# tsnorri/vcf2multialign

Measured on AMD Instinct MI355X. Metric: aligned A2M Gbases/sec, higher is better.
Workload: dtype u8

## Files before the change

vcf2multialign_amd/csrc/kernels.hpp:

```cpp
#pragma once

#include <hip/hip_runtime.h>
#include <stdint.h>

#ifdef V2M_CHECKED_BUILD
__device__ uint32_t v2m_lds_poison_seed;
#endif

namespace v2m {

typedef uint32_t u32;
typedef uint64_t u64;

constexpr int kWave = 64;
typedef u32 vec4u __attribute__((ext_vector_type(4)));
typedef vec4u vec4u_unaligned8 __attribute__((aligned(8)));

#ifdef V2M_CHECKED_BUILD
__device__ __forceinline__ u32 poison_hash(u32 seed, u32 wg, u32 i)
{
	u32 h = seed ^ (wg * 0x9E3779B1u) ^ (i * 0x85EBCA77u);
	h ^= h >> 15; h *= 0x2C1B3C6Du;
	h ^= h >> 12; h *= 0x297A2D39u;
	h ^= h >> 15;
// ... 741 lines not shown
		}
	}
	for (u32 e = 0; e < 15; ++e) {
		u32 const cg = span_hi + e;
#pragma unroll
		for (int a = 0; a < kA; ++a)
			if (col_ok[a]) emit_guarded(a, cg & 15u, cg);
	}
}
#endif


__device__ __forceinline__ uint4 expand_reference_chunk(
	char const *__restrict__ ref, u32 const *__restrict__ ref_pos, u32 const *__restrict__ aln_pos,
	u32 n_nodes, u32 L, u64 p0, char gap, unsigned char past)
{
	unsigned char bytes[16];
	if (p0 >= L) {
		u32 const w = past * 0x01010101u;
		return make_uint4(w, w, w, w);
	}
	u32 lo = 0, hi = n_nodes;
	while (hi - lo > 1) {
		u32 const mid = lo + (hi - lo) / 2;
		if (aln_pos[mid] <= p0) lo = mid; else hi = mid;
	}
	u32 n = lo;
	u32 a0 = aln_pos[n], r0 = ref_pos[n];
	u32 a1 = (n + 1 < n_nodes) ? aln_pos[n + 1] : 0xFFFFFFFFu;
	u32 r1 = (n + 1 < n_nodes) ? ref_pos[n + 1] : r0;
#pragma unroll
	for (int b = 0; b < 16; ++b) {
		u64 const p = p0 + b;
		unsigned char v = past;
		if (p < L) {
			while (p >= a1) {
				++n;
				a0 = a1; r0 = r1;
				a1 = (n + 1 < n_nodes) ? aln_pos[n + 1] : 0xFFFFFFFFu;
				r1 = (n + 1 < n_nodes) ? ref_pos[n + 1] : r0;
			}
			u32 const off = (u32) p - a0;
			v = (off < r1 - r0) ? (unsigned char) ref[r0 + off] : (unsigned char) gap;
		}
		bytes[b] = v;
	}
	uint4 o;
	o.x = bytes[0] | (bytes[1] << 8) | (bytes[2] << 16) | ((u32) bytes[3] << 24);
	o.y = bytes[4] | (bytes[5] << 8) | (bytes[6] << 16) | ((u32) bytes[7] << 24);
	o.z = bytes[8] | (bytes[9] << 8) | (bytes[10] << 16) | ((u32) bytes[11] << 24);
	o.w = bytes[12] | (bytes[13] << 8) | (bytes[14] << 16) | ((u32) bytes[15] << 24);
	return o;
}

__global__ __launch_bounds__(256) void expand_reference_row_kernel(
	char const *__restrict__ ref, u32 const *__restrict__ ref_pos, u32 const *__restrict__ aln_pos,
	u32 n_nodes, u32 L, u64 n_chunks, uint4 *__restrict__ out, char gap, u32 col_base = 0)
{
	u64 const c = (u64) blockIdx.x * blockDim.x + threadIdx.x;
	if (c >= n_chunks) return;
	u64 const p0 = col_base + c * 16;
	out[c] = expand_reference_chunk(ref, ref_pos, aln_pos, n_nodes, L, p0, gap, 0);
}

struct set_tile_tables {
	u32 const *col_begin;
	u32 const *col_end;
	u32 const *record_offset;
	u32 const *edge_end;
};

__global__ __launch_bounds__(256) void expand_reference_set_kernel(
	char const *__restrict__ ref, u32 const *__restrict__ ref_pos, u32 const *__restrict__ aln_pos,
	u32 n_nodes, set_tile_tables st, u32 n_tiles, u64 n_chunks, uint4 *__restrict__ out, char gap)
{
	u64 const c = (u64) blockIdx.x * blockDim.x + threadIdx.x;
	if (c >= n_chunks) return;
	u32 lo = 0, hi = n_tiles;
	while (hi - lo > 1) {
		u32 const mid = lo + (hi - lo) / 2;
		if ((u64) st.record_offset[mid] <= c * 16) lo = mid; else hi = mid;
	}
	u64 const p0 = (u64) st.col_begin[lo] + (c * 16 - st.record_offset[lo]);
	out[c] = expand_reference_chunk(ref, ref_pos, aln_pos, n_nodes, st.col_end[lo], p0, gap, (unsigned char) gap);
}


struct row_segments {
	u32 const *seg_offsets;
	u32 const *seg_edge_begin;
	u32 const *seg_copy;
	u64 const *assembled;
	u32 assembled_words;
};

__device__ __forceinline__ u64 load_row_word(
	u64 const *__restrict__ paths, u64 words_per_copy, row_segments const &rs, u32 row, u32 s_begin, u32 s_end, u32 wi)
{
	if (s_end - s_begin == 1) {
		u32 const copy = rs.seg_copy[s_begin];
		return (copy == 0xFFFFFFFFu) ? 0 : paths[(u64) copy * words_per_copy + wi];
	}
	return rs.assembled[(u64) row * rs.assembled_words + wi];
}

__global__ __launch_bounds__(256) void assemble_row_bits_kernel(
	u64 const *__restrict__ paths, u64 words_per_copy, row_segments rs, u64 *__restrict__ assembled, u32 n_words, u32 row_base, u32 word_base)
{
	__shared__ unsigned long long acc[256];
	u32 const row = blockIdx.y + row_base;
	u32 const s_begin = rs.seg_offsets[row], s_end = rs.seg_offsets[row + 1];
	if (s_end - s_begin <= 1) return;
	V2M_POISON_LDS(acc);
	u32 const lane = threadIdx.x & 63, wave = threadIdx.x >> 6;
	u32 const w0 = word_base + (blockIdx.x * 4 + wave) * 64;
	acc[threadIdx.x] = 0;
	__syncthreads();
	if (w0 < n_words) {
		u64 const e_lo = (u64) w0 * 64;
		u64 const e_hi = (u64) (w0 + 64 < n_words ? w0 + 64 : n_words) * 64;
		u32 lo = s_begin, hi = s_end;
		while (hi - lo > 1) {
			u32 const mid = lo + (hi - lo) / 2;
			if (rs.seg_edge_begin[mid] <= e_lo) lo = mid; else hi = mid;
		}
		for (u32 s = lo + lane; s < s_end; s += 64) {
			u64 b = rs.seg_edge_begin[s];
			if (b >= e_hi) break;
			u64 e = (s + 1 < s_end) ? rs.seg_edge_begin[s + 1] : ~0ULL;
			u32 const copy = rs.seg_copy[s];
			if (copy == 0xFFFFFFFFu) continue;
			b = b > e_lo ? b : e_lo;
			e = e < e_hi ? e : e_hi;
			if (b >= e) continue;
			u64 const *const column = paths + (u64) copy * words_per_copy;
			for (u64 wi = b >> 6; wi <= (e - 1) >> 6; ++wi) {
				u64 const base = wi * 64;
				u32 const from = b > base ? (u32) (b - base) : 0;
				u32 const to = e < base + 64 ? (u32) (e - base) : 64;
				u64 const mask = (to >= 64 ? ~0ULL : ((1ULL << to) - 1)) & ~((1ULL << from) - 1);
				u64 const v = column[wi] & mask;
				if (v) atomicOr(&acc[wave * 64 + (u32) (wi - w0)], (unsigned long long) v);
			}
		}
	}
	__syncthreads();
	if (w0 + lane < n_words) assembled[(u64) row * rs.assembled_words + w0 + lane] = acc[threadIdx.x];
}

constexpr int kResolveWordsPerThread = 8;
constexpr u32 kResolveQueueShards = 1024;
constexpr u32 kMaxBackWords = 2048;

__device__ __forceinline__ u64 resolve_word_exact(
	u64 const *__restrict__ paths, u64 words_per_copy, row_segments const &rs, u32 row, u32 s_begin, u32 s_end,
	edge_span const *__restrict__ spans, u64 const *__restrict__ overlappable,
	u32 wi, u64 w, u64 ovl_w, u32 *__restrict__ needs_serial, u32 max_back_words)
{
	u64 const ov = w & ovl_w;
	if (0 == ov) return w;
	int const b0 = __builtin_ctzll(ov);
	u32 sw = wi;
	int sb = 0;
	u64 fixed = ~ovl_w & ((1ULL << b0) - 1);
	if (fixed) {
		sb = 63 - __builtin_clzll(fixed);
	} else {
		u32 steps = 0;
		for (;;) {
			if (0 == sw) { sb = 0; break; }
			--sw;
			if (++steps > max_back_words) { atomicOr(&needs_serial[row], 1u); return w; }
			fixed = ~overlappable[sw];
			if (fixed) { sb = 63 - __builtin_clzll(fixed); break; }
		}
	}
	u64 out = (sw == wi) ? (w & ((1ULL << sb) - 1)) : 0;
	u32 cur = 0;
	for (u32 ww = sw; ww <= wi; ++ww) {
		u64 x = (ww == wi) ? w : load_row_word(paths, words_per_copy, rs, row, s_begin, s_end, ww);
		if (ww == sw) x &= ~((1ULL << sb) - 1);
		while (x) {
			constexpr int kBatch = 8;
			edge_span sp[kBatch];
			int bit[kBatch];
			bool has[kBatch];
#pragma unroll
			for (int k = 0; k < kBatch; ++k) {
				has[k] = 0 != x;
				bit[k] = has[k] ? __builtin_ctzll(x) : 0;
				x &= x - 1;
				sp[k] = spans[ww * 64u + bit[k]];
			}
#pragma unroll
			for (int k = 0; k < kBatch; ++k) {
				if (has[k] && sp[k].src >= cur) {
					cur = sp[k].tgt;
					if (ww == wi) out |= 1ULL << bit[k];
				}
			}
		}
	}
	return out;
}

__global__ __launch_bounds__(256) void resolve_effective_edges_kernel(
	u64 const *__restrict__ paths, u64 words_per_copy, u32 n_edges,
	row_segments rs, edge_span const *__restrict__ spans, u64 const *__restrict__ overlappable,
	u32 const *__restrict__ ovl_rank, u64 const *__restrict__ blocker_masks,
	u64 *__restrict__ eff, u32 n_words, u32 eff_words_per_row, u32 row_base, u32 word_base,
	u32 *__restrict__ queue, u32 *__restrict__ queue_counts , u32 shard_capacity, u32 *__restrict__ needs_serial, u32 max_back_words)
{
	u32 const row = blockIdx.x + row_base;
	u32 const shard = (blockIdx.y * gridDim.x + blockIdx.x) % kResolveQueueShards;
	u32 const s_begin = rs.seg_offsets[row], s_end = rs.seg_offsets[row + 1];
	u64 const tail_mask = (n_edges & 63) ? (1ULL << (n_edges & 63)) - 1 : ~0ULL;
	u64 const *row_words = nullptr;
	if (s_end - s_begin == 1) {
		u32 const copy = rs.seg_copy[s_begin];
		if (copy != 0xFFFFFFFFu) row_words = paths + (u64) copy * words_per_copy;
	} else {
		row_words = rs.assembled + (u64) row * rs.assembled_words;
	}
	u32 const w_first = word_base + blockIdx.y * kResolveWordsPerThread * blockDim.x + threadIdx.x;
	u64 w_all[kResolveWordsPerThread], ovl_all[kResolveWordsPerThread], mask_a[kResolveWordsPerThread], mask_b[kResolveWordsPerThread];
	u32 rank_all[kResolveWordsPerThread];
#pragma unroll
	for (int piece = 0; piece < kResolveWordsPerThread; ++piece) {
		u32 const wi = w_first + piece * blockDim.x;
		u32 const wc = wi < n_words ? wi : n_words - 1;
		w_all[piece] = row_words ? row_words[wc] : 0;
		ovl_all[piece] = overlappable[wc];
		rank_all[piece] = ovl_rank[wc];
		if (wi == (n_edges - 1) >> 6) w_all[piece] &= tail_mask;
	}
#pragma unroll
	for (int piece = 0; piece < kResolveWordsPerThread; ++piece) {
		u64 const ov = w_all[piece] & ovl_all[piece], ov2 = ov & (ov - 1);
		auto const entry = [&](u64 m) {
			return m ? rank_all[piece] + (u32) __builtin_popcountll(ovl_all[piece] & ((1ULL << __builtin_ctzll(m)) - 1)) : 0u;
		};
		mask_a[piece] = blocker_masks[entry(ov)];
		mask_b[piece] = blocker_masks[entry(ov2)];
	}
	int const lane = threadIdx.x & 63;
#pragma unroll
	for (int piece = 0; piece < kResolveWordsPerThread; ++piece) {
		u32 const wi = w_first + piece * blockDim.x;
		bool const in_range = wi < n_words;
		u64 const w = w_all[piece], ov = w & ovl_all[piece], ov2 = ov & (ov - 1);
		bool const hard = in_range && ov && ((w & mask_a[piece]) || (ov2 && ((w & mask_b[piece]) || (ov2 & (ov2 - 1)))));
		if (in_range && !hard) eff[(u64) row * eff_words_per_row + wi] = w;
		u64 const hard_lanes = __ballot(hard);
		if (hard_lanes) {
			u32 base = 0;
			if (0 == lane) base = atomicAdd(&queue_counts[shard], (u32) __builtin_popcountll(hard_lanes));
			base = __shfl(base, 0, kWave);
			if (hard) {
				u32 const slot = base + __builtin_amdgcn_mbcnt_hi((u32) (hard_lanes >> 32), __builtin_amdgcn_mbcnt_lo((u32) hard_lanes, 0));
				if (slot < shard_capacity) queue[(u64) shard * shard_capacity + slot] = (row - row_base) * n_words + wi;
				else eff[(u64) row * eff_words_per_row + wi] = resolve_word_exact(paths, words_per_copy, rs, row, s_begin, s_end, spans, overlappable, wi, w, ovl_all[piece], needs_serial, max_back_words);
			}
		}
	}
}

__global__ __launch_bounds__(256) void resolve_queued_words_kernel(
	u64 const *__restrict__ paths, u64 words_per_copy, u32 n_edges,
	row_segments rs, edge_span const *__restrict__ spans, u64 const *__restrict__ overlappable,
	u64 *__restrict__ eff, u32 n_words, u32 eff_words_per_row, u32 row_base,
	u32 const *__restrict__ queue, u32 const *__restrict__ queue_counts, u32 shard_capacity, u32 *__restrict__ needs_serial, u32 max_back_words)
{
	u32 const shard = blockIdx.x % kResolveQueueShards, part = blockIdx.x / kResolveQueueShards, parts = gridDim.x / kResolveQueueShards;
	u32 const n = queue_counts[shard] < shard_capacity ? queue_counts[shard] : shard_capacity;
	u64 const tail_mask = (n_edges & 63) ? (1ULL << (n_edges & 63)) - 1 : ~0ULL;
	for (u32 i = part * blockDim.x + threadIdx.x; i < n; i += parts * blockDim.x) {
		u32 const entry = queue[(u64) shard * shard_capacity + i];
		u32 const row = row_base + entry / n_words, wi = entry % n_words;
		u32 const s_begin = rs.seg_offsets[row], s_end = rs.seg_offsets[row + 1];
		u64 w = load_row_word(paths, words_per_copy, rs, row, s_begin, s_end, wi);
		if (wi == (n_edges - 1) >> 6) w &= tail_mask;
		eff[(u64) row * eff_words_per_row + wi] = resolve_word_exact(paths, words_per_copy, rs, row, s_begin, s_end, spans, overlappable, wi, w, overlappable[wi], needs_serial, max_back_words);
	}
}


__global__ __launch_bounds__(256) void resolve_rows_serial_kernel(
	u64 const *__restrict__ paths, u64 words_per_copy, u32 n_edges,
	row_segments rs, edge_span const *__restrict__ spans,
	u64 *__restrict__ eff, u64 eff_words_per_row, u32 n_rows, u32 const *__restrict__ needs_serial,
	u32 word_begin , u32 word_end)
{
	int const lane = threadIdx.x & 63;
	u32 const row = blockIdx.x * (blockDim.x >> 6) + (threadIdx.x >> 6);
	if (row >= n_rows) return;
	if (needs_serial && 0 == needs_serial[row]) return;

	u32 const s_begin = rs.seg_offsets[row], s_end = rs.seg_offsets[row + 1];
	u32 const n_words = (n_edges + 63) / 64;
	u64 *const eff_row = eff + (u64) row * eff_words_per_row;
	u32 cur = 0;

	for (u32 base = word_begin; base < word_end; base += 64) {
		u32 const wi = base + lane;
		u64 w = 0;
		if (wi < word_end) {
			w = load_row_word(paths, words_per_copy, rs, row, s_begin, s_end, wi);
			if (wi == n_words - 1 && (n_edges & 63))
				w &= (1ULL << (n_edges & 63)) - 1;
		}

		u32 lane_max = 0;
		for (u64 m = w; m; m &= m - 1) {
			u32 const e = wi * 64u + __builtin_ctzll(m);
			u32 const tgt = spans[e].tgt;
			lane_max = tgt > lane_max ? tgt : lane_max;
		}
		u32 incl = lane_max;
#pragma unroll
		for (int d = 1; d < 64; d <<= 1) {
			u32 const o = __shfl_up(incl, d, kWave);
			if (lane >= d) incl = o > incl ? o : incl;
		}
		u32 excl = __shfl_up(incl, 1, kWave);
		if (lane == 0) excl = 0;
		u32 const chunk_max = __shfl(incl, 63, kWave);

		u32 run = excl > cur ? excl : cur;
		bool uncertain = false;
		for (u64 m = w; m; m &= m - 1) {
			u32 const e = wi * 64u + __builtin_ctzll(m);
			edge_span const sp = spans[e];
			uncertain |= sp.src < run;
			run = sp.tgt > run ? sp.tgt : run;
		}

		u64 out = w;
		if (__any(uncertain)) {
			out = 0;
			u32 c = cur;
			u64 busy = __ballot(w != 0);
			while (busy) {
				int const j = __builtin_ctzll(busy);
				busy &= busy - 1;
				if (lane == j) {
					for (u64 m = w; m; m &= m - 1) {
						int const b = __builtin_ctzll(m);
						edge_span const sp = spans[wi * 64u + b];
						if (sp.src >= c) {
							out |= 1ULL << b;
							c = sp.tgt;
						}
					}
				}
				c = __shfl(c, j, kWave);
			}
			cur = c;
		} else {
			cur = chunk_max > cur ? chunk_max : cur;
		}
		if (wi < word_end)
			eff_row[wi] = out;
	}
}


struct tile_tables {
	u32 const *edge_begin;
	u32 const *cross_offsets;
	u32 const *cross_edges;
};

template <typename LabelPtr>
__device__ __forceinline__ void fill_patch_bytes(
	unsigned char *tile, u32 tile_base, u32 aln_begin, u32 label_len, LabelPtr label,
	u32 from, u32 to, u32 start, u32 step, char gap)
{
	for (u32 pos = from + start; pos < to; pos += step) {
		u32 const off = pos - aln_begin;
		tile[pos - tile_base] = (off < label_len) ? (unsigned char) label[off] : (unsigned char) gap;
	}
}

constexpr int kCandLds = 512;
constexpr int kLabelLds = 1024;
constexpr int kGroupRowsLds = 16;
constexpr int kEffWordsLds = kCandLds / 64 + 2;
constexpr int kLongQueueLds = 16;

struct cached_patch {
	unsigned short begin_rel;
	unsigned short span;
	unsigned short label_rel;
	unsigned short label_len;
};

struct patch_cache {
	cached_patch patch[kCandLds];
	u64 eff[kGroupRowsLds][kEffWordsLds];
	unsigned char labels[kLabelLds];
	u32 long_queue[kLongQueueLds];
	u32 long_count;
};

struct tile_job {
	u32 tile_base, tile_end;
	u32 cross_begin, n_cross, range_begin, n_range;
	u32 n_lds;
	u32 w0;
};

__device__ __forceinline__ void load_eff_cache(
	patch_cache &pc, tile_job const &job, u64 const *__restrict__ eff, u64 eff_words_per_row, u32 first_row, u32 n_rows, int t)
{
	if (0 == job.n_lds) return;
	u32 const nw = ((job.range_begin + job.n_lds - 1) >> 6) - job.w0 + 1;
	u32 const rows = n_rows < (u32) kGroupRowsLds ? n_rows : (u32) kGroupRowsLds;
	for (u32 i = t; i < rows * nw; i += kSpliceThreads)
		pc.eff[i / nw][i % nw] = eff[(u64) (first_row + i / nw) * eff_words_per_row + job.w0 + i % nw];
}

template <bool kWindow = false, bool kSet = false>
__device__ __forceinline__ void load_patch_cache(
	patch_cache &pc, tile_job &job, tile_tables const &tt, edge_patch const *__restrict__ patches, char const *__restrict__ labels,
	u64 const *__restrict__ eff, u64 eff_words_per_row, u32 tile, u32 row_begin, u32 n_group_rows, int t, u32 col_base = 0, u32 col_end = 0,
	set_tile_tables const st = set_tile_tables{})
{
	if (kSet) {
		job.tile_base = st.col_begin[tile];
		job.tile_end = st.col_end[tile];
	} else {
		job.tile_base = (kWindow ? col_base : 0u) + tile * (u32) kTileBytes;
		job.tile_end = (kWindow && col_end - job.tile_base < (u32) kTileBytes) ? col_end : job.tile_base + kTileBytes;
	}
	job.cross_begin = tt.cross_offsets[tile];
	job.n_cross = tt.cross_offsets[tile + 1] - job.cross_begin;
	job.range_begin = tt.edge_begin[tile];
	job.n_range = (kSet ? st.edge_end[tile] : tt.edge_begin[tile + 1]) - job.range_begin;
	job.n_lds = job.n_range < (u32) kCandLds ? job.n_range : (u32) kCandLds;
	job.w0 = job.range_begin >> 6;
	if (job.n_lds) {
		u32 const label_base = patches[job.range_begin].label_begin;
		for (u32 i = t; i < job.n_lds; i += kSpliceThreads) {
			edge_patch const p = patches[job.range_begin + i];
			u32 const span = p.aln_end - p.aln_begin, rel = p.label_begin - label_base;
			cached_patch c;
			c.begin_rel = (unsigned short) (p.aln_begin - job.tile_base);
			c.span = span < 0xFFFFu ? (unsigned short) span : (unsigned short) 0xFFFF;
			bool const label_ok = rel + p.label_len <= (u32) kLabelLds;
			c.label_rel = label_ok ? (unsigned short) rel : (unsigned short) 0xFFFF;
			c.label_len = label_ok ? (unsigned short) p.label_len : (unsigned short) 0;
			pc.patch[i] = c;
		}
		edge_patch const last = patches[job.range_begin + job.n_lds - 1];
		u32 const label_span = last.label_begin + last.label_len - label_base;
		u32 const label_len = label_span < (u32) kLabelLds ? label_span : (u32) kLabelLds;
		for (u32 i = t; i < label_len; i += kSpliceThreads)
			pc.labels[i] = (unsigned char) labels[label_base + i];
	}
	load_eff_cache(pc, job, eff, eff_words_per_row, row_begin, n_group_rows, t);
	if (t == 0) pc.long_count = 0;
}

struct tile_patch {
	u32 edge;
	u32 aln_begin;
	u32 from, to;
	u32 label_len;
	u32 label_begin;
	bool in_lds;
};

__device__ __forceinline__ u32 candidate_edge(tile_job const &job, tile_tables const &tt, u32 i)
{
	return (i < job.n_cross) ? tt.cross_edges[job.cross_begin + i] : job.range_begin + (i - job.n_cross);
}

__device__ __forceinline__ bool candidate_in_lds(tile_job const &job, u32 i)
{
	return i >= job.n_cross && i - job.n_cross < job.n_lds;
}

template <bool kWindow = false>
__device__ __forceinline__ tile_patch candidate_patch(
	patch_cache const &pc, tile_job const &job, edge_patch const *__restrict__ patches, u32 i, u32 e, bool cached)
{
	u32 const tile_end = kWindow ? job.tile_end : job.tile_base + kTileBytes;
	cached_patch c{};
	if (cached) {
		c = pc.patch[i - job.n_cross];
		cached = c.span != 0xFFFF && c.label_rel != 0xFFFF;
	}
	tile_patch tp;
	tp.edge = e;
	if (cached) {
		tp.aln_begin = tp.from = job.tile_base + c.begin_rel;
		tp.to = tp.from + c.span < tile_end ? tp.from + c.span : tile_end;
		tp.label_len = c.label_len;
		tp.label_begin = c.label_rel;
		tp.in_lds = true;
	} else {
		edge_patch const p = patches[e];
		tp.aln_begin = p.aln_begin;
		tp.from = p.aln_begin > job.tile_base ? p.aln_begin : job.tile_base;
		tp.to = p.aln_end < tile_end ? p.aln_end : tile_end;
		tp.label_len = p.label_len;
		tp.label_begin = p.label_begin;
		tp.in_lds = false;
	}
	return tp;
}

__device__ __forceinline__ bool candidate_effective(
	patch_cache const &pc, tile_job const &job, tile_tables const &tt, u64 const *__restrict__ eff_row, u32 local_row, u32 i,
	u32 &e, bool &cached)
// ... 790 lines not shown
```

vcf2multialign_amd/csrc/v2m_hip.hip:

```cpp

#include <hip/hip_runtime.h>

#include <algorithm>
#include <atomic>
#include <chrono>
#include <condition_variable>
#include <cstdarg>
#include <cstdio>
#include <cstdlib>
#include <cstring>
#include <memory>
#include <mutex>
#include <string>
#include <thread>
#include <utility>
#include <vector>

#include <type_traits>

#include "../../include/v2m_hip.h"
#include "kernels.hpp"
#include "founder_kernels.hpp"
#include "bgzf_kernels.hpp"
#include "vcf_kernels.hpp"
// ... 21 lines not shown
	if (!p || !n) return hipSuccess;
	hipError_t st(hipDeviceSynchronize());
	if (hipSuccess != st) return st;
	u64 const words(n / 4);
	unsigned const blocks(unsigned(std::min<u64>(4096, words / 256 + 1)));
	hipLaunchKernelGGL(v2m::poison_fill_kernel, dim3(blocks), dim3(256), 0, 0, static_cast<unsigned char *>(p), u64(n), g_poison_seed.load(), poison_mix(g_poison_salt++));
	if (hipSuccess != (st = hipGetLastError())) return st;
	return hipDeviceSynchronize();
}

void poison_host(void *p, size_t n)
{
	if (!p) return;
	u32 const salt(poison_mix(g_poison_salt++ ^ g_poison_seed.load()));
	unsigned char *const b(static_cast<unsigned char *>(p));
	for (size_t i(0); i < n / 4; ++i) { u32 const w(poison_mix(salt ^ u32(i) * 0x9E3779B1u)); std::memcpy(b + 4 * i, &w, 4); }
	for (size_t i(n / 4 * 4); i < n; ++i) b[i] = (unsigned char) poison_mix(salt + u32(i));
}
#define V2M_POISON_HOST(p, n) poison_host((p), (n))
#else
#define V2M_POISON_HOST(p, n) ((void) 0)
#endif

struct dev_buf {
	void *p{};
	size_t bytes{};
	dev_buf() = default;
	dev_buf(dev_buf const &) = delete;
	dev_buf &operator=(dev_buf const &) = delete;
	~dev_buf() { reset(); }
	void reset() { if (p) (void) hipFree(p); p = nullptr; bytes = 0; }
	hipError_t ensure(size_t n)
	{
		if (n <= bytes) return hipSuccess;
		reset();
		if (0 == n) return hipSuccess;
		hipError_t const st(hipMalloc(&p, n));
		if (hipSuccess == st) bytes = n; else p = nullptr;
#ifdef V2M_CHECKED_BUILD
		if (hipSuccess == st) return poison_device(p, n);
#endif
		return st;
	}
	template <typename T> T *as() const { return static_cast<T *>(p); }
};

struct scratch_buf : dev_buf {
	hipError_t ensure(size_t n)
	{
		bool const fresh(n > bytes);
		hipError_t const st(dev_buf::ensure(n));
#ifdef V2M_CHECKED_BUILD
		if (hipSuccess == st && !fresh) return poison_device(p, bytes);
#else
		(void) fresh;
#endif
		return st;
	}
};

struct pinned_buf {
	void *p{};
	size_t bytes{};
	~pinned_buf() { reset(); }
	void reset() { if (p) (void) hipHostFree(p); p = nullptr; bytes = 0; }
	hipError_t ensure(size_t n)
	{
		if (n <= bytes) return hipSuccess;
		reset();
		if (0 == n) return hipSuccess;
		hipError_t const st(hipHostMalloc(&p, n, hipHostMallocDefault));
		if (hipSuccess == st) bytes = n; else p = nullptr;
		return st;
	}
	template <typename T> T *as() const { return static_cast<T *>(p); }
};

struct event_pair { hipEvent_t begin{}, end{}; };

}


struct held_ring_state {
	std::mutex mutex;
	std::condition_variable released;
};

struct v2m_row_hold {
	pinned_buf host;
	hipEvent_t copied{};
	uint64_t outstanding{};
	held_ring_state *ring{};
};


struct word_range { u64 restart, lo, hi, stride; };

struct row_view {
	u64 begin{}, end{};
	u64 max_unaligned{};
	u32 n_tiles{};
	dev_buf d_template, d_template0;
	bool has_template0{};
	dev_buf d_edge_begin, d_cross_offsets, d_cross_edges;
	word_range words{};
	u64 length() const { return end - begin; }
};


struct v2m_ctx {
	int device{};
	u32 n_cus{256};
	hipStream_t stream{};
	hipStream_t copy_stream{};
	std::string err;

	bool profiling{};
	std::vector<event_pair> events[V2M_KERNEL_COUNT];
	std::vector<event_pair> free_events;

	bool has_graph{};
	u64 n_nodes{}, n_edges{}, ref_len{}, aligned_len{}, label_bytes{};
	bool has_nul_byte{};
	std::vector<u32> h_csum;
	std::vector<u32> h_tgt_prefix_max;
	dev_buf d_ref, d_ref_pos, d_aln_pos, d_spans, d_patches, d_labels, d_overlappable;
	dev_buf d_ovl_rank, d_blocker_masks;
	std::vector<u32> h_aln_pos, h_tile_edge_begin, h_cross_offsets, h_cross_edges;
	std::vector<v2m::edge_patch> h_patches;
	std::vector<u64> h_overlappable;

	row_view whole, window;
	bool windowed{};
	row_view &view() { return set_call ? set.view : windowed ? window : whole; }
	row_view const &view() const { return set_call ? set.view : windowed ? window : whole; }

	struct window_set {
		row_view view;
		u64 n_windows{}, pitch{}, mean_tile_bytes{};
		std::vector<u32> lengths;
		dev_buf d_col_begin, d_col_end, d_record_offset, d_edge_end, d_tile_window, d_first_tile, d_slot_offset32;
	} set;
	bool has_set{}, set_call{};
	scratch_buf d_set_tile_offsets, d_set_lengths[2];
	int set_lengths_slot{};

	u64 const *d_paths{};
	dev_buf owned_paths;
	dev_buf d_slice_src;
	u64 path_rows{}, path_cols{};
	u64 path_pitch{};
	dev_buf d_by_edge;
	bool by_edge_valid{};

	struct transpose_pick { u64 rows, cols, src_pitch, dst_pitch; std::string kernel; };
	std::vector<transpose_pick> transpose_choice;

	int store_mode{-1};
	int unaligned_store_mode{-1};
	std::string info;

	pinned_buf h_row_stage[2];
	hipEvent_t ev_row_stage[2]{};
	bool row_stage_in_flight[2]{};
	int row_stage_next{};
	scratch_buf d_resolve_queue, d_resolve_count;
	scratch_buf d_eff, d_row_bits, d_seg_offsets, d_seg_edge_begin, d_seg_copy, d_sums, d_lengths, d_needs_serial, d_tile_counts, d_row_lengths;
	scratch_buf ring[2];
	held_ring_state held_state;
	std::vector<std::unique_ptr<v2m_row_hold>> host_slots;
	pinned_buf trials_stage[2];
	scratch_buf d_bgzf_slots, d_bgzf_sizes, d_bgzf_offsets, d_bgzf_table, d_bgzf_dense[2], d_bgzf_in;
	pinned_buf h_bgzf_table[2];
	hipEvent_t ev_compute[2]{};
	scratch_buf d_inflate_in[2], d_inflate_out[2], d_inflate_status[2];
	hipEvent_t ev_inflate_in[2]{};
	dev_buf d_vcf_text[2];
	scratch_buf d_vcf_in, d_vcf_status, d_vcf_tiles, d_vcf_tile_offsets, d_vcf_line_start, d_vcf_lines, d_vcf_gt_off, d_vcf_flags, d_vcf_tmp_begin,
		d_vcf_tmp_columns, d_vcf_totals, d_vcf_heads, d_vcf_columns, d_vcf_layout, d_vcf_wanted;
};


namespace {

int fail(v2m_ctx *ctx, int code, char const *fmt, ...)
{
	char buf[512];
	va_list ap;
	va_start(ap, fmt);
	std::vsnprintf(buf, sizeof(buf), fmt, ap);
	va_end(ap);
	if (ctx) ctx->err = buf; else g_create_error = buf;
	return code;
}

#define V2M_HIP_TRY(ctx, expr)                                                              \
	do {                                                                                    \
		hipError_t const st_ = (expr);                                                      \
		if (hipSuccess != st_) {                                                            \
			int const code_ = (hipErrorOutOfMemory == st_) ? V2M_ERR_OUT_OF_MEMORY : V2M_ERR_HIP; \
			return fail(ctx, code_, "%s failed: %s", #expr, hipGetErrorString(st_));       \
		}                                                                                   \
	} while (0)


struct timed_launch {
	v2m_ctx *ctx;
	int kernel;
	event_pair ev{};
	bool active{};

	timed_launch(v2m_ctx *c, int k) : ctx(c), kernel(k)
	{
		if (!ctx->profiling) return;
		if (!ctx->free_events.empty()) { ev = ctx->free_events.back(); ctx->free_events.pop_back(); }
		else if (hipSuccess != hipEventCreate(&ev.begin) || hipSuccess != hipEventCreate(&ev.end)) return;
		active = (hipSuccess == hipEventRecord(ev.begin, ctx->stream));
	}
	~timed_launch()
	{
		if (!active) return;
		(void) hipEventRecord(ev.end, ctx->stream);
		ctx->events[kernel].push_back(ev);
	}
};


template <typename T>
int upload_vec(v2m_ctx *ctx, dev_buf &dst, std::vector<T> const &src, size_t min_bytes = 16)
{
	size_t const bytes(std::max(src.size() * sizeof(T), min_bytes));
	V2M_HIP_TRY(ctx, dst.ensure(bytes));
	if (!src.empty())
		V2M_HIP_TRY(ctx, hipMemcpyAsync(dst.p, src.data(), src.size() * sizeof(T), hipMemcpyHostToDevice, ctx->stream));
	return V2M_OK;
}


struct scoped_events {
	std::vector<hipEvent_t> ev;
	~scoped_events() { for (auto e : ev) (void) hipEventDestroy(e); }
	hipError_t create(std::size_t n)
	{
		for (std::size_t i(0); i < n; ++i) {
			hipEvent_t e{};
			hipError_t const st(hipEventCreate(&e));
			if (hipSuccess != st) return st;
			ev.push_back(e);
		}
		return hipSuccess;
	}
	hipEvent_t operator[](std::size_t i) const { return ev[i]; }
};

struct scoped_profiling_off {
	v2m_ctx *ctx;
	bool was;
	explicit scoped_profiling_off(v2m_ctx *c) : ctx(c), was(c->profiling) { c->profiling = false; }
	~scoped_profiling_off() { ctx->profiling = was; }
};


struct xcd_grid { unsigned blocks; u32 items_per_xcd; };

bool make_xcd_grid(u64 n_items, bool xcd, xcd_grid &g)
{
	u64 const per((n_items + 7) / 8), blocks(xcd ? per * 8 : n_items);
	if (0 == n_items || blocks > 0x7FFFFFFFull) return false;
	g.blocks = unsigned(blocks);
	g.items_per_xcd = xcd ? u32(per) : 0u;
	return true;
}

u32 rows_fastest_for(int order, u64 n_row_panels, u64 n_col_panels)
{
	if (1 == order) return 1;
	if (2 == order) return 0;
	return n_row_panels <= n_col_panels ? 1u : 0u;
}

template <int kR, int kC>
int launch_transpose_shape(v2m_ctx *ctx, u64 const *d_src, u64 SW, u64 DW, u64 SP, u64 DP, u64 *d_dst, bool xcd, int order)
{
	u64 const P((SW + kR - 1) / kR), Q((DW + kC - 1) / kC);
	xcd_grid g;
	if (P > 0xFFFFFFFFull || Q > 0xFFFFFFFFull || !make_xcd_grid(P * Q, xcd, g))
		return fail(ctx, V2M_ERR_UNSUPPORTED, "matrix too large for one transpose launch (%llu x %llu bits)", (unsigned long long) (SW * 64), (unsigned long long) (DW * 64));
	{
		timed_launch tl(ctx, V2M_KERNEL_TRANSPOSE);
		hipLaunchKernelGGL((v2m::transpose_bits_kernel<kR, kC>), dim3(g.blocks), dim3(v2m::kTrThreads), 0, ctx->stream, d_src, d_dst, SW, DW, SP, DP, u32(P), u32(Q), g.items_per_xcd, rows_fastest_for(order, P, Q));
	}
	V2M_HIP_TRY(ctx, hipGetLastError());
	return V2M_OK;
}

template <int kDepth, int kSlabCols, int kWaves = 4, int kTsR = 16, int kTsC = 16, bool kLean = true>
int launch_transpose_stream(v2m_ctx *ctx, u64 const *d_src, u64 SW, u64 DW, u64 SP, u64 DP, u64 *d_dst, bool xcd, int order)
{
	u64 const P((SW + kTsR - 1) / kTsR), Q((DW + kTsC - 1) / kTsC);
	xcd_grid g;
	if (P > 0xFFFFFFFFull || Q > 0xFFFFFFFFull || !make_xcd_grid(P * Q, xcd, g)) return fail(ctx, V2M_ERR_UNSUPPORTED, "matrix too large for one transpose launch");
	{
		timed_launch tl(ctx, V2M_KERNEL_TRANSPOSE);
		hipLaunchKernelGGL((v2m::transpose_bits_stream_kernel<kDepth, kSlabCols, kWaves, kTsR, kTsC, kLean>), dim3(g.blocks), dim3(64 * kWaves), 0, ctx->stream, d_src, d_dst, SW, DW, SP, DP, u32(P), u32(Q), g.items_per_xcd, rows_fastest_for(order, P, Q));
	}
	V2M_HIP_TRY(ctx, hipGetLastError());
// ... 247 lines not shown
	return launch_transpose_named(ctx, names[pick], d_src, SW, DW, SP, DP, d_dst);
}


struct prepared_rows {
	u32 *seg_offsets{};
	u32 *seg_edge_begin{};
	u32 *seg_copy{};
	u64 n_rows{}, n_segments{};
	bool any_switching_row{};
};

int prepare_rows(v2m_ctx *ctx, v2m_row_batch const *rows, u64 row_begin, u64 row_end, prepared_rows &out)
{
	u64 const n_rows(row_end - row_begin);
	u64 max_segments(n_rows);
	if (rows->cut_offsets) {
		for (u64 r(row_begin); r < row_end; ++r) {
			if (rows->cut_offsets[r + 1] < rows->cut_offsets[r])
				return fail(ctx, V2M_ERR_INVALID_ARGUMENT, "cut_offsets decrease at row %llu", (unsigned long long) r);
			max_segments += rows->cut_offsets[r + 1] - rows->cut_offsets[r];
		}
	}
	if (max_segments >= 0xFFFFFFFFull)
		return fail(ctx, V2M_ERR_UNSUPPORTED, "row batch has too many cut segments (%llu) for one call", (unsigned long long) max_segments);
	auto const pad([](u64 n) { return (n * sizeof(u32) + 63) & ~u64(63); });
	int const area(ctx->row_stage_next);
	if (ctx->row_stage_in_flight[area]) {
		V2M_HIP_TRY(ctx, hipEventSynchronize(ctx->ev_row_stage[area]));
		ctx->row_stage_in_flight[area] = false;
	}
	V2M_HIP_TRY(ctx, ctx->h_row_stage[area].ensure(pad(n_rows + 1) + 2 * pad(max_segments)));
	char *const base(static_cast<char *>(ctx->h_row_stage[area].p));
	V2M_POISON_HOST(base, pad(n_rows + 1) + 2 * pad(max_segments));
	out.seg_offsets = reinterpret_cast<u32 *>(base);
	out.seg_edge_begin = reinterpret_cast<u32 *>(base + pad(n_rows + 1));
	out.seg_copy = reinterpret_cast<u32 *>(base + pad(n_rows + 1) + pad(max_segments));
	out.n_rows = n_rows;
	out.any_switching_row = false;

	out.seg_offsets[0] = 0;
	for (u64 r(row_begin); r < row_end; ++r) {
		u64 const c_begin(rows->cut_offsets ? rows->cut_offsets[r] : 0), c_end(rows->cut_offsets ? rows->cut_offsets[r + 1] : 0);
		u64 const n_seg(c_begin == c_end ? 1 : (c_end - c_begin) + (0 != rows->cut_nodes[c_begin] ? 1 : 0));
		out.seg_offsets[r - row_begin + 1] = u32(out.seg_offsets[r - row_begin] + n_seg);
		out.any_switching_row = out.any_switching_row || n_seg > 1;
	}
	out.n_segments = out.seg_offsets[n_rows];

	struct row_error { int code{V2M_OK}; std::string text; };
	auto const fill_row([&](u64 r, row_error &err) {
		auto const failed([&](int code, char const *fmt, unsigned long long a, unsigned long long b = 0) {
			char buf[256];
			std::snprintf(buf, sizeof(buf), fmt, a, b);
			err.code = code;
			err.text = buf;
		});
		u64 const c_begin(rows->cut_offsets ? rows->cut_offsets[r] : 0), c_end(rows->cut_offsets ? rows->cut_offsets[r + 1] : 0);
		u32 n(out.seg_offsets[r - row_begin]);
		if (c_begin == c_end) {
			if (!rows->copy_index) return failed(V2M_ERR_INVALID_ARGUMENT, "row %llu has no cuts and rows->copy_index is NULL", r);
			u32 const copy(rows->copy_index[r]);
			if (copy != V2M_PLOIDY_MAX && (!ctx->d_paths || copy >= ctx->path_cols))
				return failed(V2M_ERR_INVALID_ARGUMENT, "row %llu: chromosome copy %llu is outside the path matrix", r, copy);
			out.seg_edge_begin[n] = 0;
			out.seg_copy[n] = copy;
			return;
		}
		u64 prev(0);
		for (u64 k(c_begin); k < c_end; ++k) {
			u64 const node(rows->cut_nodes[k]);
			u32 const copy(rows->cut_copies[k]);
			if (node >= ctx->n_nodes) return failed(V2M_ERR_PRECONDITION, "row %llu: cut node %llu does not exist", r, node);
			if (k > c_begin && node <= prev) return failed(V2M_ERR_PRECONDITION, "row %llu: cut nodes must be strictly increasing", r);
			if (copy != V2M_PLOIDY_MAX && (!ctx->d_paths || copy >= ctx->path_cols))
				return failed(V2M_ERR_INVALID_ARGUMENT, "row %llu: chromosome copy %llu is outside the path matrix", r, copy);
			u32 const first_edge(ctx->h_csum[node]);
			if (node > 0 && ctx->h_tgt_prefix_max[first_edge] > node)
				return failed(V2M_ERR_PRECONDITION, "row %llu: cut node %llu lies inside the span of an ALT edge", r, node);
			if (k == c_begin && node != 0) {
				out.seg_edge_begin[n] = 0;
				out.seg_copy[n] = V2M_PLOIDY_MAX;
				++n;
			}
			out.seg_edge_begin[n] = first_edge;
			out.seg_copy[n] = copy;
			++n;
			prev = node;
		}
	});
	std::vector<row_error> errors(n_rows);
	unsigned const n_threads(out.n_segments >= (u64(1) << 20) ? unsigned(std::min<u64>(n_rows, 8)) : 1u);
	if (n_threads <= 1) {
		for (u64 r(row_begin); r < row_end; ++r) { fill_row(r, errors[r - row_begin]); if (V2M_OK != errors[r - row_begin].code) break; }
	}
	else {
		std::atomic<u64> next(row_begin);
		auto const work([&] { for (u64 r; (r = next.fetch_add(1)) < row_end;) fill_row(r, errors[r - row_begin]); });
		std::vector<std::thread> pool;
		for (unsigned t(1); t < n_threads; ++t) pool.emplace_back(work);
		work();
		for (auto &t : pool) t.join();
	}
	for (auto const &e : errors) if (V2M_OK != e.code) return fail(ctx, e.code, "%s", e.text.c_str());
	return V2M_OK;
}


int forced_store_mode(bool unaligned)
{
	if (unaligned) {
		char const *const e = std::getenv("V2M_UNALIGNED_STORE");
		if (e && 0 == std::strcmp(e, "plain")) return 0;
		if (e && 0 == std::strcmp(e, "nt")) return 1;
		return -1;
	}
	char const *e = std::getenv("V2M_NT_STORES");
	if (!(e && *e)) return -1;
	return std::atoi(e) != 0 ? 1 : 0;
}

u32 rows_per_group_for(u64 n_rows)
{
	char const *e = std::getenv("V2M_ROWS_PER_GROUP");
	int const v((e && *e) ? std::atoi(e) : 0);
	if (v > 0) return u32(std::min(v, 256));
	return u32(std::min<u64>(32, std::max<u64>(1, n_rows)));
}


u32 rows_per_group_for_set(u64 n_rows, u64 mean_tile_bytes)
{
	char const *e = std::getenv("V2M_ROWS_PER_GROUP");
	if (e && *e && std::atoi(e) > 0) return rows_per_group_for(n_rows);
	u64 const by_bytes(32 * u64(v2m::kTileBytes) / std::max<u64>(1, mean_tile_bytes));
	return u32(std::min<u64>(std::max<u64>(1, n_rows), std::min<u64>(256, std::max<u64>(32, by_bytes))));
}


int expand_reference(v2m_ctx *ctx, row_view const &v, dev_buf &dst, char gap)
{
	u64 const n_chunks(u64(v.n_tiles) * v2m::kTileChunks);
	V2M_HIP_TRY(ctx, dst.ensure(n_chunks * 16));
	{
		timed_launch tl(ctx, V2M_KERNEL_TEMPLATE);
		hipLaunchKernelGGL(v2m::expand_reference_row_kernel, dim3(unsigned((n_chunks + 255) / 256)), dim3(256), 0, ctx->stream,
			ctx->d_ref.as<char>(), ctx->d_ref_pos.as<u32>(), ctx->d_aln_pos.as<u32>(), u32(ctx->n_nodes), u32(v.end), n_chunks, dst.as<uint4>(), gap, u32(v.begin));
	}
	V2M_HIP_TRY(ctx, hipGetLastError());
	return V2M_OK;
}


int resolve_slice(v2m_ctx *ctx, v2m_row_batch const *rows, u64 row_begin, u64 row_end)
{
	u64 const n_rows(row_end - row_begin);
	word_range const wr(ctx->view().words);
	u64 const eff_words(wr.stride), n_words(wr.hi);
	if (0 == ctx->n_edges) return V2M_OK;

	prepared_rows pr;
	if (int const rc = prepare_rows(ctx, rows, row_begin, row_end, pr)) return rc;
	if (wr.lo >= wr.hi) return V2M_OK;
	auto const upload([&](scratch_buf &dst, u32 const *src, u64 count) -> int {
		V2M_HIP_TRY(ctx, dst.ensure(std::max<size_t>(count * sizeof(u32), 16)));
		if (count) V2M_HIP_TRY(ctx, hipMemcpyAsync(dst.p, src, count * sizeof(u32), hipMemcpyHostToDevice, ctx->stream));
		return V2M_OK;
	});
	int const stage(ctx->row_stage_next);
	ctx->row_stage_in_flight[stage] = true;
	ctx->row_stage_next ^= 1;
	int upload_rc(upload(ctx->d_seg_offsets, pr.seg_offsets, n_rows + 1));
	if (!upload_rc) upload_rc = upload(ctx->d_seg_edge_begin, pr.seg_edge_begin, pr.n_segments);
	if (!upload_rc) upload_rc = upload(ctx->d_seg_copy, pr.seg_copy, pr.n_segments);
	hipError_t const recorded(hipEventRecord(ctx->ev_row_stage[stage], ctx->stream));
	if (upload_rc) return upload_rc;
	V2M_HIP_TRY(ctx, recorded);
	V2M_HIP_TRY(ctx, ctx->d_eff.ensure(n_rows * eff_words * sizeof(u64)));
	V2M_HIP_TRY(ctx, ctx->d_needs_serial.ensure(n_rows * sizeof(u32)));
	V2M_HIP_TRY(ctx, hipMemsetAsync(ctx->d_needs_serial.p, 0, n_rows * sizeof(u32), ctx->stream));

	bool const any_switching_row(pr.any_switching_row);
	if (any_switching_row) V2M_HIP_TRY(ctx, ctx->d_row_bits.ensure(n_rows * eff_words * sizeof(u64)));

	u64 *const d_eff(ctx->d_eff.as<u64>() - wr.restart);
	u64 *const d_row_bits(any_switching_row ? ctx->d_row_bits.as<u64>() - wr.restart : nullptr);
	v2m::row_segments rs{ctx->d_seg_offsets.as<u32>(), ctx->d_seg_edge_begin.as<u32>(), ctx->d_seg_copy.as<u32>(), d_row_bits, u32(eff_words)};
	char const *const back_env(std::getenv("V2M_MAX_BACK_WORDS"));
	u32 const max_back_words((back_env && *back_env) ? u32(std::strtoul(back_env, nullptr, 10)) : v2m::kMaxBackWords);
	char const *const capacity_env(std::getenv("V2M_RESOLVE_QUEUE_CAPACITY"));
	bool const capacity_forced(capacity_env && *capacity_env);
	{
		timed_launch tl(ctx, V2M_KERNEL_RESOLVE);
		u64 const rows_per_launch(std::max<u64>(1, std::min<u64>(65535, 0xFFFFFFFFull / std::max<u64>(1, n_words))));
		u64 const assembled_words(n_words - wr.restart), resolved_words(n_words - wr.lo);
		for (u64 r0(0); r0 < n_rows; r0 += rows_per_launch) {
			u64 const nr(std::min<u64>(rows_per_launch, n_rows - r0));
			if (any_switching_row)
				for (u64 y0(0); y0 < nr; y0 += 65535)
					hipLaunchKernelGGL(v2m::assemble_row_bits_kernel, dim3(unsigned((assembled_words + 255) / 256), unsigned(std::min<u64>(65535, nr - y0))), dim3(256), 0, ctx->stream,
						ctx->d_paths, ctx->path_pitch, rs, d_row_bits, u32(n_words), u32(r0 + y0), u32(wr.restart));
			u64 const shard_capacity(capacity_forced ? std::min<u64>(std::strtoull(capacity_env, nullptr, 10), (u64(1) << 28) / v2m::kResolveQueueShards)
				: std::max<u64>(256, std::min<u64>(nr * resolved_words, u64(1) << 28) / v2m::kResolveQueueShards));
			V2M_HIP_TRY(ctx, ctx->d_resolve_queue.ensure(shard_capacity * v2m::kResolveQueueShards * sizeof(u32)));
			V2M_HIP_TRY(ctx, ctx->d_resolve_count.ensure(v2m::kResolveQueueShards * sizeof(u32)));
			V2M_HIP_TRY(ctx, hipMemsetAsync(ctx->d_resolve_count.p, 0, v2m::kResolveQueueShards * sizeof(u32), ctx->stream));
			for (u64 piece0(0), pieces((resolved_words + 256 * v2m::kResolveWordsPerThread - 1) / (256 * v2m::kResolveWordsPerThread)); piece0 < pieces; piece0 += 65535)
				hipLaunchKernelGGL(v2m::resolve_effective_edges_kernel, dim3(unsigned(nr), unsigned(std::min<u64>(65535, pieces - piece0))), dim3(256), 0, ctx->stream,
					ctx->d_paths, ctx->path_pitch, u32(ctx->n_edges), rs, ctx->d_spans.as<v2m::edge_span>(), ctx->d_overlappable.as<u64>(),
					ctx->d_ovl_rank.as<u32>(), ctx->d_blocker_masks.as<u64>(),
					d_eff, u32(n_words), u32(eff_words), u32(r0), u32(wr.lo + piece0 * 256 * v2m::kResolveWordsPerThread),
					ctx->d_resolve_queue.as<u32>(), ctx->d_resolve_count.as<u32>(), u32(shard_capacity), ctx->d_needs_serial.as<u32>(), max_back_words);
			hipLaunchKernelGGL(v2m::resolve_queued_words_kernel, dim3(2 * v2m::kResolveQueueShards), dim3(256), 0, ctx->stream,
				ctx->d_paths, ctx->path_pitch, u32(ctx->n_edges), rs, ctx->d_spans.as<v2m::edge_span>(), ctx->d_overlappable.as<u64>(),
				d_eff, u32(n_words), u32(eff_words), u32(r0),
				ctx->d_resolve_queue.as<u32>(), ctx->d_resolve_count.as<u32>(), u32(shard_capacity), ctx->d_needs_serial.as<u32>(), max_back_words);
		}
		hipLaunchKernelGGL(v2m::resolve_rows_serial_kernel, dim3(unsigned((n_rows + 3) / 4)), dim3(256), 0, ctx->stream,
			ctx->d_paths, ctx->path_pitch, u32(ctx->n_edges), rs, ctx->d_spans.as<v2m::edge_span>(),
			d_eff, eff_words, u32(n_rows), ctx->d_needs_serial.as<u32>(), u32(wr.restart), u32(n_words));
	}
	V2M_HIP_TRY(ctx, hipGetLastError());
	return V2M_OK;
}


struct splice_grid {
	u32 rows_per_group, n_groups, tile_run;
	u64 n_blocks;
};

u32 tile_run_for(u32 n_tiles)
{
	char const *e = std::getenv("V2M_TILE_RUN");
	int const v((e && *e) ? std::atoi(e) : 0);
	u32 const run(v > 0 ? u32(v) : 64u);
	return std::max<u32>(1, std::min(run, n_tiles));
}

int make_grid(v2m_ctx *ctx, u64 n_rows, splice_grid &g)
{
	g.rows_per_group = ctx->set_call ? rows_per_group_for_set(n_rows, ctx->set.mean_tile_bytes) : rows_per_group_for(n_rows);
	g.n_groups = u32((n_rows + g.rows_per_group - 1) / g.rows_per_group);
	g.n_blocks = u64(ctx->view().n_tiles) * g.n_groups;
	g.tile_run = tile_run_for(ctx->view().n_tiles);
	if (g.n_blocks > 0x7FFFFFFFull)
		return fail(ctx, V2M_ERR_UNSUPPORTED, "splice grid too large (%llu workgroups); use smaller batches", (unsigned long long) g.n_blocks);
	return V2M_OK;
}


template <typename F>
int store_flavour_launch(v2m_ctx *ctx, bool unaligned, u64 n_rows, u64 bytes, F const &launch)
{
	int &slot(unaligned ? ctx->unaligned_store_mode : ctx->store_mode);
	int mode(forced_store_mode(unaligned));
	if (mode < 0) mode = slot;
	if (mode < 0 && bytes >= (u64(1) << 30)) {
		scoped_events ev;
		V2M_HIP_TRY(ctx, ev.create(5));
		V2M_HIP_TRY(ctx, hipEventRecord(ev[0], ctx->stream));
		for (int i(0); i < 4; ++i) {
			launch(0 == (i & 1));
			V2M_HIP_TRY(ctx, hipEventRecord(ev[i + 1], ctx->stream));
		}
		V2M_HIP_TRY(ctx, hipStreamSynchronize(ctx->stream));
		float t[4];
		for (int i(0); i < 4; ++i) V2M_HIP_TRY(ctx, hipEventElapsedTime(&t[i], ev[i], ev[i + 1]));
		float const nt_ms(std::min(t[0], t[2])), plain_ms(std::min(t[1], t[3]));
		slot = nt_ms <= plain_ms ? 1 : 0;
		char buf[160];
		std::snprintf(buf, sizeof(buf), "%s splice stores: %s (calibrated on %llu rows: nontemporal %.3f ms, plain %.3f ms)",
			unaligned ? "unaligned" : "aligned", slot ? "nontemporal" : "plain", (unsigned long long) n_rows, nt_ms, plain_ms);
		if (unaligned && ctx->info.size() > 2000) ctx->info.clear();
		if (!ctx->info.empty()) ctx->info += "; ";
		ctx->info += buf;
		mode = slot;
	}
	if (mode < 0) mode = 1;
	{
		timed_launch tl(ctx, unaligned ? V2M_KERNEL_SPLICE_UNALIGNED : V2M_KERNEL_SPLICE_ALIGNED);
		launch(0 != mode);
	}
	V2M_HIP_TRY(ctx, hipGetLastError());
	return V2M_OK;
}


v2m::set_tile_tables set_tables(v2m_ctx const *ctx)
{
	auto const &s(ctx->set);
	return {s.d_col_begin.as<u32>(), s.d_col_end.as<u32>(), s.d_record_offset.as<u32>(), s.d_edge_end.as<u32>()};
}

int expand_reference_set(v2m_ctx *ctx, dev_buf &dst, char gap);


int splice_aligned_slice(v2m_ctx *ctx, v2m_row_batch const *rows, u64 row_begin, u64 row_end, char *d_out, u64 row_pitch)
{
	u64 const n_rows(row_end - row_begin);
	if (0 == n_rows || 0 == ctx->aligned_len) return V2M_OK;
	if (int const rc = resolve_slice(ctx, rows, row_begin, row_end)) return rc;

	row_view const &v(ctx->view());
	splice_grid g;
	if (int const rc = make_grid(ctx, n_rows, g)) return rc;
	v2m::tile_tables const tt{v.d_edge_begin.as<u32>(), v.d_cross_offsets.as<u32>(), v.d_cross_edges.as<u32>()};
	u64 const store_limit((v.length() + 15) & ~u64(15));
	auto const launch([&](bool nt) {
		auto const go([&](auto kernel, auto... window) {
			hipLaunchKernelGGL(kernel, dim3(unsigned(g.n_blocks)), dim3(v2m::kSpliceThreads), 0, ctx->stream,
				v.d_template.as<v2m::vec4u>(), ctx->d_eff.as<u64>() - v.words.restart, v.words.stride, tt, ctx->d_patches.as<v2m::edge_patch>(), ctx->d_labels.as<char>(),
				d_out, row_pitch, u32(n_rows), g.rows_per_group, g.n_groups, v.n_tiles, g.tile_run, store_limit, '-', window...);
		});
		if (ctx->set_call) {
			auto const go_set([&](auto kernel) {
				hipLaunchKernelGGL(kernel, dim3(unsigned(g.n_blocks)), dim3(v2m::kSpliceThreads), 0, ctx->stream,
					v.d_template.as<v2m::vec4u>(), ctx->d_eff.as<u64>() - v.words.restart, v.words.stride, tt, set_tables(ctx), ctx->d_patches.as<v2m::edge_patch>(), ctx->d_labels.as<char>(),
					d_out, row_pitch, u32(n_rows), g.rows_per_group, g.n_groups, v.n_tiles, g.tile_run, '-');
			});
			if (nt) go_set(v2m::splice_aligned_set_kernel<true>);
			else go_set(v2m::splice_aligned_set_kernel<false>);
		}
		else if (ctx->windowed) {
			if (nt) go(v2m::splice_aligned_window_kernel<true>, u32(v.begin), u32(v.end));
			else go(v2m::splice_aligned_window_kernel<false>, u32(v.begin), u32(v.end));
		}
		else if (nt) go(v2m::splice_aligned_kernel<true>);
		else go(v2m::splice_aligned_kernel<false>);
	});
	return store_flavour_launch(ctx, false, n_rows, n_rows * v.length(), launch);
}


int splice_unaligned_slice(v2m_ctx *ctx, v2m_row_batch const *rows, u64 row_begin, u64 row_end, char *d_out, u64 row_pitch)
{
	u64 const n_rows(row_end - row_begin);
	if (0 == n_rows) return V2M_OK;
	V2M_HIP_TRY(ctx, ctx->d_row_lengths.ensure(n_rows * sizeof(u64)));
	if (0 == ctx->aligned_len) {
		V2M_HIP_TRY(ctx, hipMemsetAsync(ctx->d_row_lengths.p, 0, n_rows * sizeof(u64), ctx->stream));
		return V2M_OK;
	}
	row_view &v(ctx->view());
	bool const set(ctx->set_call);
	if (!v.has_template0) {
		if (int const rc = set ? expand_reference_set(ctx, v.d_template0, 0) : expand_reference(ctx, v, v.d_template0, 0)) return rc;
		v.has_template0 = true;
	}
	if (int const rc = resolve_slice(ctx, rows, row_begin, row_end)) return rc;

	splice_grid g;
	if (int const rc = make_grid(ctx, n_rows, g)) return rc;
	V2M_HIP_TRY(ctx, ctx->d_tile_counts.ensure(n_rows * v.n_tiles * sizeof(u32)));
	if (set) {
		V2M_HIP_TRY(ctx, ctx->d_set_tile_offsets.ensure(n_rows * v.n_tiles * sizeof(u32)));
		V2M_HIP_TRY(ctx, ctx->d_set_lengths[ctx->set_lengths_slot].ensure(n_rows * ctx->set.n_windows * sizeof(u32)));
	}
	bool const windowed(ctx->windowed);
	v2m::tile_tables const tt{v.d_edge_begin.as<u32>(), v.d_cross_offsets.as<u32>(), v.d_cross_edges.as<u32>()};
	u64 const *const d_eff(ctx->d_eff.as<u64>() - v.words.restart);
	{
		char const *const ce(std::getenv("V2M_COUNT_ROWS_PER_GROUP"));
		u32 const count_rows(u32(std::min<u64>(std::max<u64>(1, n_rows), (ce && *ce && std::atoi(ce) > 0) ? u64(std::min(std::atoi(ce), int(v2m::kCountRowsMax))) : u64(v2m::kCountRowsMax))));
		u32 const count_groups(u32((n_rows + count_rows - 1) / count_rows));
		timed_launch tl(ctx, V2M_KERNEL_UNALIGNED_COUNT);
		auto const count([&](auto kernel, auto... window) {
			hipLaunchKernelGGL(kernel, dim3(unsigned(u64(v.n_tiles) * count_groups)), dim3(v2m::kSpliceThreads), 0, ctx->stream,
				v.d_template0.as<v2m::vec4u>(), d_eff, v.words.stride, tt, ctx->d_patches.as<v2m::edge_patch>(), ctx->d_labels.as<char>(),
				ctx->d_tile_counts.as<u32>(), v.n_tiles, u32(n_rows), count_rows, count_groups, g.tile_run, window...);
		});
		if (set)
			hipLaunchKernelGGL(v2m::count_unaligned_set_kernel, dim3(unsigned(u64(v.n_tiles) * count_groups)), dim3(v2m::kSpliceThreads), 0, ctx->stream,
				v.d_template0.as<v2m::vec4u>(), d_eff, v.words.stride, tt, set_tables(ctx), ctx->d_patches.as<v2m::edge_patch>(), ctx->d_labels.as<char>(),
				ctx->d_tile_counts.as<u32>(), v.n_tiles, u32(n_rows), count_rows, count_groups, g.tile_run);
		else if (windowed) count(v2m::count_unaligned_window_kernel, u32(v.begin), u32(v.end));
		else count(v2m::count_unaligned_kernel);
		hipLaunchKernelGGL(v2m::scan_tile_counts_kernel, dim3(unsigned(n_rows)), dim3(256), 0, ctx->stream,
			ctx->d_tile_counts.as<u32>(), v.n_tiles, ctx->d_row_lengths.as<u64>());
		if (set)
			hipLaunchKernelGGL(v2m::scan_window_set_kernel, dim3(unsigned(n_rows)), dim3(256), 0, ctx->stream,
				ctx->d_tile_counts.as<u32>(), ctx->d_row_lengths.as<u64>(), v.n_tiles, u32(ctx->set.n_windows),
				ctx->set.d_first_tile.as<u32>(), ctx->set.d_tile_window.as<u32>(), ctx->set.d_slot_offset32.as<u32>(),
				ctx->d_set_tile_offsets.as<u32>(), ctx->d_set_lengths[ctx->set_lengths_slot].as<u32>());
	}
	auto const launch([&](bool nt) {
		auto const go([&](auto kernel, auto... window) {
			hipLaunchKernelGGL(kernel, dim3(unsigned(g.n_blocks)), dim3(v2m::kSpliceThreads), 0, ctx->stream,
				v.d_template0.as<v2m::vec4u>(), d_eff, v.words.stride, tt, ctx->d_patches.as<v2m::edge_patch>(), ctx->d_labels.as<char>(),
				ctx->d_tile_counts.as<u32>(), v.n_tiles, d_out, row_pitch, u32(n_rows), g.rows_per_group, g.n_groups, g.tile_run, window...);
		});
		if (set) {
			auto const go_set([&](auto kernel) {
				hipLaunchKernelGGL(kernel, dim3(unsigned(g.n_blocks)), dim3(v2m::kSpliceThreads), 0, ctx->stream,
					v.d_template0.as<v2m::vec4u>(), d_eff, v.words.stride, tt, set_tables(ctx), ctx->d_patches.as<v2m::edge_patch>(), ctx->d_labels.as<char>(),
					ctx->d_set_tile_offsets.as<u32>(), v.n_tiles, d_out, row_pitch, u32(n_rows), g.rows_per_group, g.n_groups, g.tile_run);
			});
			if (nt) go_set(v2m::splice_unaligned_set_kernel<true>);
			else go_set(v2m::splice_unaligned_set_kernel<false>);
			return;
		}
		if (windowed) {
			if (nt) go(v2m::splice_unaligned_window_kernel<true>, u32(v.begin), u32(v.end));
			else go(v2m::splice_unaligned_window_kernel<false>, u32(v.begin), u32(v.end));
			return;
		}
#ifdef V2M_TUNING_BUILD
		static int const flavour([] { char const *const e(std::getenv("V2M_UNALIGNED_KERNEL")); return !e ? 0 : 0 == std::strcmp(e, "wave") ? 1 : 0 == std::strcmp(e, "shared64") ? 2 : 0; }());
		if (1 == flavour) { if (nt) go(v2m::splice_unaligned_per_wave_kernel<true>); else go(v2m::splice_unaligned_per_wave_kernel<false>); return; }
		if (2 == flavour) { if (nt) go(v2m::splice_unaligned_kernel<true, 64>); else go(v2m::splice_unaligned_kernel<false, 64>); return; }
#endif
		if (nt) go(v2m::splice_unaligned_kernel<true>);
		else go(v2m::splice_unaligned_kernel<false>);
	});
	return store_flavour_launch(ctx, true, n_rows, n_rows * ((set || windowed) ? v.length() : ctx->ref_len), launch);
}


int check_batch(v2m_ctx *ctx, v2m_row_batch const *rows, u32 flags)
{
	if (!ctx) return V2M_ERR_INVALID_ARGUMENT;
	if (!rows) return fail(ctx, V2M_ERR_INVALID_ARGUMENT, "rows is NULL");
	if (flags & ~(V2M_SPLICE_UNALIGNED | V2M_SPLICE_BGZF)) return fail(ctx, V2M_ERR_INVALID_ARGUMENT, "unknown flags 0x%x", flags);
	if (!ctx->has_graph) return fail(ctx, V2M_ERR_STATE, "no graph uploaded");
	if (rows->n_rows && !rows->copy_index && !rows->cut_offsets) return fail(ctx, V2M_ERR_INVALID_ARGUMENT, "rows->copy_index is NULL");
	if (rows->cut_offsets && rows->cut_offsets[rows->n_rows] && (!rows->cut_nodes || !rows->cut_copies))
		return fail(ctx, V2M_ERR_INVALID_ARGUMENT, "cut arrays are NULL");
	if (rows->n_rows >= 0xFFFFFFFFull) return fail(ctx, V2M_ERR_UNSUPPORTED, "too many rows in one batch");
	if (ctx->d_by_edge.p) { ctx->d_by_edge.reset(); ctx->by_edge_valid = false; }
	if ((flags & V2M_SPLICE_UNALIGNED) && ctx->has_nul_byte)
		return fail(ctx, V2M_ERR_UNSUPPORTED, "the reference sequence or an ALT label holds a NUL byte, which the unaligned kernels use as their padding marker; aligned mode keeps such bytes");
	return V2M_OK;
}


struct slice_plan { u64 pitch, rows_per_slice, n_slices, slot_bytes; };

slice_plan plan_slices(v2m_ctx const *ctx, u64 n_rows, bool unaligned, u64 max_rows_per_slice = ~u64(0))
{
	slice_plan p;
	p.pitch = ctx->set_call ? ctx->set.pitch : unaligned ? ((v2m_max_unaligned_length(ctx) + 255) & ~u64(255)) : v2m_min_row_pitch(ctx);
	char const *const slot_env(std::getenv("V2M_RING_SLOT_BYTES"));
	u64 const slot_default(n_rows * p.pitch < (u64(8) << 30) ? (u64(128) << 20) : (u64(512) << 20));
	u64 const slot_target((slot_env && *slot_env) ? std::strtoull(slot_env, nullptr, 10) : slot_default);
	p.rows_per_slice = std::max<u64>(1, std::min<u64>({n_rows, slot_target / p.pitch, max_rows_per_slice}));
	p.n_slices = (n_rows + p.rows_per_slice - 1) / p.rows_per_slice;
	p.slot_bytes = p.rows_per_slice * p.pitch;
	return p;
}

int ensure_host_slots(v2m_ctx *ctx, u64 n, u64 bytes)
{
	while (ctx->host_slots.size() < n) {
		std::unique_ptr<v2m_row_hold> slot(new v2m_row_hold);
		slot->ring = &ctx->held_state;
		V2M_HIP_TRY(ctx, hipEventCreateWithFlags(&slot->copied, hipEventDisableTiming));
		ctx->host_slots.push_back(std::move(slot));
	}
	for (u64 i(0); i < n; ++i) V2M_HIP_TRY(ctx, ctx->host_slots[i]->host.ensure(bytes));
	return V2M_OK;
}

void wait_released(v2m_ctx *ctx, v2m_row_hold &slot)
{
	std::unique_lock<std::mutex> lock(ctx->held_state.mutex);
	ctx->held_state.released.wait(lock, [&] { return 0 == slot.outstanding; });
}



u64 bgzf_pieces(u64 n) { return (n + v2m::kBgzfBlockBytes - 1) / v2m::kBgzfBlockBytes; }

int bgzf_encode_rows(v2m_ctx *ctx, char const *d_rows, u64 pitch, u64 const *d_lengths, u64 length, u64 max_len, u64 n_rows, char *d_dense)
{
	u64 const per_row(std::max<u64>(1, bgzf_pieces(max_len)));
	u64 const n_blocks(n_rows * per_row);
	if (n_blocks > 0x7FFFFFFFull || per_row > 0xFFFFFFFFull)
		return fail(ctx, V2M_ERR_UNSUPPORTED, "BGZF grid too large (%llu blocks); use smaller batches", (unsigned long long) n_blocks);
	V2M_HIP_TRY(ctx, ctx->d_bgzf_slots.ensure(n_blocks * v2m::kBgzfSlotBytes));
	V2M_HIP_TRY(ctx, ctx->d_bgzf_sizes.ensure(n_blocks * sizeof(u32)));
	V2M_HIP_TRY(ctx, ctx->d_bgzf_offsets.ensure(n_blocks * sizeof(u64)));
	V2M_HIP_TRY(ctx, ctx->d_bgzf_table.ensure((n_rows + 1) * sizeof(u64)));
	{
		timed_launch tl(ctx, V2M_KERNEL_BGZF);
		hipLaunchKernelGGL(v2m::bgzf_deflate_kernel, dim3(unsigned(n_blocks)), dim3(v2m::kBgzfThreads), 0, ctx->stream,
			d_rows, pitch, d_lengths, length, u32(per_row), ctx->d_bgzf_slots.as<char>(), ctx->d_bgzf_sizes.as<u32>());
		hipLaunchKernelGGL(v2m::bgzf_scan_kernel, dim3(1), dim3(v2m::kBgzfScanThreads), 0, ctx->stream,
			ctx->d_bgzf_sizes.as<u32>(), n_blocks, u32(per_row), n_rows, ctx->d_bgzf_offsets.as<u64>(), ctx->d_bgzf_table.as<u64>());
		hipLaunchKernelGGL(v2m::bgzf_compact_kernel, dim3(unsigned(n_blocks)), dim3(256), 0, ctx->stream,
			ctx->d_bgzf_slots.as<char>(), ctx->d_bgzf_sizes.as<u32>(), ctx->d_bgzf_offsets.as<u64>(), d_dense);
	}
	V2M_HIP_TRY(ctx, hipGetLastError());
	return V2M_OK;
}


int splice_rows_bgzf(v2m_ctx *ctx, v2m_row_batch const *rows, bool unaligned, v2m_sink_fn sink, void *user)
{
	u64 const L(ctx->view().length());
	u64 const max_len(unaligned ? v2m_max_unaligned_length(ctx) : L);
	u64 const member_slots_per_row(std::max<u64>(1, bgzf_pieces(max_len)) * v2m::kBgzfSlotBytes);
	slice_plan const p(plan_slices(ctx, rows->n_rows, unaligned, (u64(1) << 30) / member_slots_per_row));
	u64 const pitch(p.pitch), rows_per_slice(p.rows_per_slice), n_slices(p.n_slices);
	u64 const dense_bytes(rows_per_slice * v2m_bgzf_bound(max_len));
	int const n_buffers(n_slices > 1 ? 2 : 1);
	for (int i(0); i < n_buffers; ++i) {
		V2M_HIP_TRY(ctx, ctx->ring[i].ensure(p.slot_bytes));
		V2M_HIP_TRY(ctx, ctx->d_bgzf_dense[i].ensure(dense_bytes));
		V2M_HIP_TRY(ctx, ctx->h_bgzf_table[i].ensure((rows_per_slice + 1) * sizeof(u64)));
	}
	if (int const rc = ensure_host_slots(ctx, n_buffers, dense_bytes)) return rc;
	std::vector<u64> extents[2];
	auto const slice_rows([&](u64 s, u64 &r0, u64 &r1) { r0 = s * rows_per_slice; r1 = std::min(rows->n_rows, r0 + rows_per_slice); });

	auto const launch([&](u64 s) -> int {
		int const b(int(s & 1));
		u64 r0, r1;
		slice_rows(s, r0, r1);
		if (s >= 2) V2M_HIP_TRY(ctx, hipStreamWaitEvent(ctx->stream, ctx->host_slots[b]->copied, 0));
		V2M_HIP_TRY(ctx, ctx->ring[b].ensure(p.slot_bytes));
		V2M_HIP_TRY(ctx, ctx->d_bgzf_dense[b].ensure(dense_bytes));
		if (int const rc = unaligned
				? splice_unaligned_slice(ctx, rows, r0, r1, ctx->ring[b].as<char>(), pitch)
				: splice_aligned_slice(ctx, rows, r0, r1, ctx->ring[b].as<char>(), pitch))
			return rc;
		if (int const rc = bgzf_encode_rows(ctx, ctx->ring[b].as<char>(), pitch, unaligned ? ctx->d_row_lengths.as<u64>() : nullptr, L, max_len, r1 - r0, ctx->d_bgzf_dense[b].as<char>()))
			return rc;
		V2M_HIP_TRY(ctx, hipMemcpyAsync(ctx->h_bgzf_table[b].p, ctx->d_bgzf_table.p, (r1 - r0 + 1) * sizeof(u64), hipMemcpyDeviceToHost, ctx->stream));
		V2M_HIP_TRY(ctx, hipEventRecord(ctx->ev_compute[b], ctx->stream));
		return V2M_OK;
	});
	auto const issue_copy([&](u64 s) -> int {
		int const b(int(s & 1));
		u64 r0, r1;
		slice_rows(s, r0, r1);
		V2M_HIP_TRY(ctx, hipEventSynchronize(ctx->ev_compute[b]));
		u64 const *const table(ctx->h_bgzf_table[b].as<u64>());
		extents[b].assign(table, table + (r1 - r0 + 1));
		pinned_buf &host(ctx->host_slots[b]->host);
		if (extents[b].back() > host.bytes)
			return fail(ctx, V2M_ERR_HIP, "BGZF members of rows %llu.. exceed their bound", (unsigned long long) r0);
		V2M_POISON_HOST(host.p, extents[b].back());
		if (extents[b].back())
			V2M_HIP_TRY(ctx, hipMemcpyAsync(host.p, ctx->d_bgzf_dense[b].p, extents[b].back(), hipMemcpyDeviceToHost, ctx->copy_stream));
		V2M_HIP_TRY(ctx, hipEventRecord(ctx->host_slots[b]->copied, ctx->copy_stream));
		return V2M_OK;
	});
	auto const drain([&](u64 s) -> int {
// ... 147 lines not shown
		case 2: launch(std::integral_constant<int, 2>{}); return;
		case 3: launch(std::integral_constant<int, 3>{}); return;
		case 4: launch(std::integral_constant<int, 4>{}); return;
		case 5: launch(std::integral_constant<int, 5>{}); return;
		case 6: launch(std::integral_constant<int, 6>{}); return;
		case 7: launch(std::integral_constant<int, 7>{}); return;
		case 8: launch(std::integral_constant<int, 8>{}); return;
		case 9: case 10: launch(std::integral_constant<int, 10>{}); return;
		case 11: case 12: launch(std::integral_constant<int, 12>{}); return;
		default: break;
	}
	if constexpr (kMaxPer > 12) {
		if (per <= 16) launch(std::integral_constant<int, 16>{});
		else launch(std::integral_constant<int, 20>{});
	}
}

}


namespace {

char const *inflate_status_text(u32 st)
{
	static char const *const text[v2m::kInflateStatusCount] = {"ok", "invalid block type", "stored block lengths do not match (LEN != ~NLEN)",
		"too many length or distance symbols (HLIT > 286 or HDIST > 30)", "invalid code-length code (over-subscribed, incomplete or undecodable)",
		"invalid code-length repeat (no previous length, or past HLIT + HDIST)", "invalid literal/length code (over-subscribed or incomplete)",
		"invalid distance code (over-subscribed or incomplete)", "no end-of-block code", "invalid literal/length symbol",
		"invalid distance symbol", "distance too far back", "output longer than ISIZE", "the deflate stream reads past the payload",
		"output shorter than ISIZE", "CRC-32 mismatch", "bad framing"};
	return st < v2m::kInflateStatusCount ? text[st] : "unknown status";
}

unsigned char const kBgzfEofMember[28] = {0x1f, 0x8b, 8, 4, 0, 0, 0, 0, 0, 0xff, 6, 0, 0x42, 0x43, 2, 0, 0x1b, 0, 3, 0, 0, 0, 0, 0, 0, 0, 0, 0};

struct bgzf_members {
	std::vector<u64> offsets;
	std::vector<u32> isize;
	u64 bytes{};
	bool ends_with_eof{};
};

int walk_error(std::string &what, int code, char const *fmt, ...)
{
	char buf[320];
	va_list ap;
	va_start(ap, fmt);
	std::vsnprintf(buf, sizeof(buf), fmt, ap);
	va_end(ap);
	what = buf;
	return code;
}

int bgzf_walk(unsigned char const *src, u64 n, bgzf_members &out, std::string &what)
{
	auto const le16([&](u64 i) { return u32(src[i]) | (u32(src[i + 1]) << 8); });
	auto const le32([&](u64 i) { return le16(i) | (le16(i + 2) << 16); });
	u32 const head_bytes(v2m::kBgzfHeaderBytes), foot_bytes(v2m::kBgzfFooterBytes);
	out = bgzf_members{};
	u64 pos(0);
	while (pos < n) {
		unsigned long long const at(pos), left(n - pos);
		if (left < 2 || 0x1f != src[pos] || 0x8b != src[pos + 1])
			return walk_error(what, V2M_ERR_INVALID_ARGUMENT, "BGZF member at compressed offset %llu: no gzip magic (1f 8b)", at);
		bool const bgzf_header(left >= 16 && 8 == src[pos + 2] && 4 == src[pos + 3] && 6 == le16(pos + 10) && 'B' == src[pos + 12] && 'C' == src[pos + 13]
			&& 2 == le16(pos + 14));
		if (!bgzf_header) {
			if (0 == pos && left >= 4 && 8 == src[2] && 0 == (src[3] & 0xe0))
				return walk_error(what, V2M_ERR_UNSUPPORTED, "the input is gzip but not BGZF (its first member has no BC extra subfield); recompress it with bgzip");
			if (left < 16) return walk_error(what, V2M_ERR_INVALID_ARGUMENT, "BGZF member at compressed offset %llu: truncated header (%llu bytes left)", at, left);
			return walk_error(what, V2M_ERR_INVALID_ARGUMENT, "BGZF member at compressed offset %llu: not a BGZF header (1f 8b 08 04, XLEN 6, one BC subfield of SLEN 2)", at);
		}
		if (left < head_bytes) return walk_error(what, V2M_ERR_INVALID_ARGUMENT, "BGZF member at compressed offset %llu: truncated header (%llu bytes left)", at, left);
		unsigned long long const size(le16(pos + 16) + 1ull);
		if (size < head_bytes + foot_bytes)
			return walk_error(what, V2M_ERR_INVALID_ARGUMENT, "BGZF member at compressed offset %llu: BSIZE %llu is shorter than a header and footer", at, size - 1);
		if (size > left)
			return walk_error(what, V2M_ERR_INVALID_ARGUMENT, "BGZF member at compressed offset %llu: BSIZE says %llu bytes, the input ends %llu bytes later (truncated)", at, size, left);
		u32 const isize(le32(pos + size - 4));
		if (isize > v2m::kBgzfSlotBytes)
			return walk_error(what, V2M_ERR_INVALID_ARGUMENT, "BGZF member at compressed offset %llu: ISIZE %llu is above 65536", at, (unsigned long long) isize);
		out.offsets.push_back(pos);
		out.isize.push_back(isize);
		out.bytes += isize;
		out.ends_with_eof = sizeof(kBgzfEofMember) == size && 0 == std::memcmp(src + pos, kBgzfEofMember, size);
		pos += size;
	}
	out.offsets.push_back(n);
	return V2M_OK;
}

void host_copy(void *dst, void const *src, u64 n)
{
	u64 const piece(u64(8) << 20);
	unsigned const k(unsigned(std::min<u64>(8, n / piece)));
	if (k < 2) { std::memcpy(dst, src, n); return; }
	u64 const share((n / k + 4095) & ~u64(4095));
	std::vector<std::thread> pool;
	for (unsigned t(1); t < k; ++t) {
		u64 const a(std::min(n, t * share)), b(std::min(n, a + share));
		if (a < b) pool.emplace_back([=] { std::memcpy(static_cast<char *>(dst) + a, static_cast<char const *>(src) + a, b - a); });
	}
	std::memcpy(dst, src, std::min(n, share));
	for (auto &th : pool) th.join();
}

}


extern "C" {

uint32_t v2m_abi_version(void) { return V2M_ABI_VERSION; }

int v2m_ctx_create(int device_id, v2m_ctx **ctx_out)
{
	if (!ctx_out) return fail(nullptr, V2M_ERR_INVALID_ARGUMENT, "ctx_out is NULL");
	*ctx_out = nullptr;
	int count(0);
	hipError_t st(hipGetDeviceCount(&count));
	if (hipSuccess != st || 0 == count)
		return fail(nullptr, V2M_ERR_NO_DEVICE, "no HIP device available (%s); this library has no CPU fallback", hipSuccess != st ? hipGetErrorString(st) : "device count is 0");
	if (device_id < 0 || device_id >= count)
		return fail(nullptr, V2M_ERR_INVALID_ARGUMENT, "device %d out of range (%d devices)", device_id, count);
	hipDeviceProp_t prop;
	st = hipGetDeviceProperties(&prop, device_id);
	if (hipSuccess != st) return fail(nullptr, V2M_ERR_HIP, "hipGetDeviceProperties: %s", hipGetErrorString(st));
	if (0 != std::strncmp(prop.gcnArchName, "gfx950", 6))
		return fail(nullptr, V2M_ERR_NO_DEVICE, "device %d is %s; this library is built for gfx950 (MI355X) only", device_id, prop.gcnArchName);
	st = hipSetDevice(device_id);
	if (hipSuccess != st) return fail(nullptr, V2M_ERR_HIP, "hipSetDevice: %s", hipGetErrorString(st));
#ifdef V2M_CHECKED_BUILD
	{
		char const *const e(std::getenv("V2M_POISON_SEED"));
		u32 const seed((e && *e) ? u32(std::strtoul(e, nullptr, 0)) : 0x9E3779B9u);
		g_poison_seed = seed;
		st = hipMemcpyToSymbol(HIP_SYMBOL(v2m_lds_poison_seed), &seed, sizeof(seed));
		if (hipSuccess != st) return fail(nullptr, V2M_ERR_HIP, "hipMemcpyToSymbol(v2m_lds_poison_seed): %s", hipGetErrorString(st));
	}
#endif

	auto *ctx(new v2m_ctx);
	ctx->device = device_id;
	if (prop.multiProcessorCount > 0) ctx->n_cus = u32(prop.multiProcessorCount);
	if (hipSuccess != (st = hipStreamCreateWithFlags(&ctx->stream, hipStreamNonBlocking))
		|| hipSuccess != (st = hipStreamCreateWithFlags(&ctx->copy_stream, hipStreamNonBlocking))) {
		delete ctx;
		return fail(nullptr, V2M_ERR_HIP, "hipStreamCreate: %s", hipGetErrorString(st));
	}
	for (int i(0); i < 2 && hipSuccess == st; ++i) {
		st = hipEventCreateWithFlags(&ctx->ev_compute[i], hipEventDisableTiming);
		if (hipSuccess == st) st = hipEventCreateWithFlags(&ctx->ev_row_stage[i], hipEventDisableTiming);
		if (hipSuccess == st) st = hipEventCreateWithFlags(&ctx->ev_inflate_in[i], hipEventDisableTiming);
	}
	if (hipSuccess != st) {
		std::string const what(hipGetErrorString(st));
		v2m_ctx_destroy(ctx);
		return fail(nullptr, V2M_ERR_HIP, "hipEventCreateWithFlags: %s", what.c_str());
	}
#ifdef V2M_CHECKED_BUILD
	char seed_info[64];
	std::snprintf(seed_info, sizeof(seed_info), "checked build: poison seed 0x%08x", g_poison_seed.load());
	ctx->info = seed_info;
#endif
	*ctx_out = ctx;
	return V2M_OK;
}

void v2m_ctx_destroy(v2m_ctx *ctx)
{
	if (!ctx) return;
	(void) hipSetDevice(ctx->device);
	(void) hipStreamSynchronize(ctx->stream);
	(void) hipStreamSynchronize(ctx->copy_stream);
	for (auto &v : ctx->events) for (auto &e : v) { (void) hipEventDestroy(e.begin); (void) hipEventDestroy(e.end); }
	for (auto &e : ctx->free_events) { (void) hipEventDestroy(e.begin); (void) hipEventDestroy(e.end); }
	for (int i(0); i < 2; ++i) {
		if (ctx->ev_compute[i]) (void) hipEventDestroy(ctx->ev_compute[i]);
		if (ctx->ev_row_stage[i]) (void) hipEventDestroy(ctx->ev_row_stage[i]);
		if (ctx->ev_inflate_in[i]) (void) hipEventDestroy(ctx->ev_inflate_in[i]);
	}
	for (auto &slot : ctx->host_slots) if (slot && slot->copied) (void) hipEventDestroy(slot->copied);
	(void) hipStreamDestroy(ctx->stream);
	(void) hipStreamDestroy(ctx->copy_stream);
	delete ctx;
}

const char *v2m_last_error(const v2m_ctx *ctx)
{
	return ctx ? ctx->err.c_str() : g_create_error.c_str();
}

int v2m_ctx_synchronize(v2m_ctx *ctx)
{
	if (!ctx) return V2M_ERR_INVALID_ARGUMENT;
	V2M_HIP_TRY(ctx, hipStreamSynchronize(ctx->stream));
	V2M_HIP_TRY(ctx, hipStreamSynchronize(ctx->copy_stream));
	return V2M_OK;
}

void *v2m_ctx_stream(v2m_ctx *ctx) { return ctx ? (void *) ctx->stream : nullptr; }

const char *v2m_ctx_info(const v2m_ctx *ctx) { return ctx ? ctx->info.c_str() : ""; }



int v2m_transpose_bits_device(v2m_ctx *ctx, const void *d_src_words, uint64_t n_rows, uint64_t n_cols, void *d_dst_words)
{
	if (!ctx) return V2M_ERR_INVALID_ARGUMENT;
	if (0 == n_cols) return V2M_OK;
	if (n_rows % 64 || n_cols % 64)
		return fail(ctx, V2M_ERR_PRECONDITION, "matrix dimensions must be multiples of 64 (got %llu x %llu)", (unsigned long long) n_rows, (unsigned long long) n_cols);
	if (0 == n_rows) return V2M_OK;
	if (!d_src_words || !d_dst_words) return fail(ctx, V2M_ERR_INVALID_ARGUMENT, "NULL matrix pointer");
	if (((uintptr_t) d_src_words | (uintptr_t) d_dst_words) & 7) return fail(ctx, V2M_ERR_INVALID_ARGUMENT, "matrix pointers must be 8-byte aligned");
	V2M_HIP_TRY(ctx, hipSetDevice(ctx->device));
	return launch_transpose(ctx, static_cast<u64 const *>(d_src_words), n_rows, n_cols, static_cast<u64 *>(d_dst_words));
}

int v2m_transpose_bits(v2m_ctx *ctx, const uint64_t *src_words, uint64_t n_rows, uint64_t n_cols, uint64_t *dst_words)
{
	if (!ctx) return V2M_ERR_INVALID_ARGUMENT;
	if (0 == n_cols) return V2M_OK;
	if (n_rows % 64 || n_cols % 64)
		return fail(ctx, V2M_ERR_PRECONDITION, "matrix dimensions must be multiples of 64 (got %llu x %llu)", (unsigned long long) n_rows, (unsigned long long) n_cols);
	if (0 == n_rows) return V2M_OK;
	if (!src_words || !dst_words) return fail(ctx, V2M_ERR_INVALID_ARGUMENT, "NULL matrix pointer");
	V2M_HIP_TRY(ctx, hipSetDevice(ctx->device));
	size_t const bytes(n_rows / 64 * n_cols * sizeof(u64));
	dev_buf src, dst;
	V2M_HIP_TRY(ctx, src.ensure(bytes));
	V2M_HIP_TRY(ctx, dst.ensure(bytes));
	V2M_HIP_TRY(ctx, hipMemcpyAsync(src.p, src_words, bytes, hipMemcpyHostToDevice, ctx->stream));
	if (int const rc = launch_transpose(ctx, src.as<u64>(), n_rows, n_cols, dst.as<u64>())) return rc;
	V2M_HIP_TRY(ctx, hipMemcpyAsync(dst_words, dst.p, bytes, hipMemcpyDeviceToHost, ctx->stream));
	V2M_HIP_TRY(ctx, hipStreamSynchronize(ctx->stream));
	return V2M_OK;
}



int v2m_upload_graph(v2m_ctx *ctx, const v2m_graph_view *g, const char *ref_seq, uint64_t ref_len)
{
	if (!ctx) return V2M_ERR_INVALID_ARGUMENT;
	if (!g) return fail(ctx, V2M_ERR_INVALID_ARGUMENT, "graph is NULL");
	u64 const N(g->node_count), E(g->edge_count);
	if (0 == N) return fail(ctx, V2M_ERR_PRECONDITION, "a variant graph has at least the source node");
	if (!g->reference_positions || !g->aligned_positions || !g->alt_edge_count_csum) return fail(ctx, V2M_ERR_INVALID_ARGUMENT, "NULL node array");
	if (E && (!g->alt_edge_targets || !g->alt_edge_label_offsets)) return fail(ctx, V2M_ERR_INVALID_ARGUMENT, "NULL edge array");
	if (ref_len && !ref_seq) return fail(ctx, V2M_ERR_INVALID_ARGUMENT, "ref_seq is NULL");
	if (g->paths_by_chrom_copy_and_edge && (g->path_rows % 64 || g->path_cols % 64 || g->path_rows < E))
		return fail(ctx, V2M_ERR_PRECONDITION, "path matrix must be (>= edge_count) x copies with both dimensions multiples of 64");
	V2M_HIP_TRY(ctx, hipSetDevice(ctx->device));

	u64 const limit32(0xFFFFFFFFull - 2 * v2m::kTileBytes);
	u64 const L(g->aligned_positions[N - 1]);
	if (N >= limit32 || E >= limit32 || L >= limit32 || ref_len >= limit32)
		return fail(ctx, V2M_ERR_UNSUPPORTED, "graph does not fit 32-bit device indices (nodes %llu, edges %llu, aligned length %llu)", (unsigned long long) N, (unsigned long long) E, (unsigned long long) L);

	std::vector<u32> ref_pos(N), aln_pos(N), csum(N + 1);
	if (0 != g->reference_positions[0] || 0 != g->aligned_positions[0])
		return fail(ctx, V2M_ERR_PRECONDITION, "node 0 must be at reference and aligned position 0");
	for (u64 n(0); n < N; ++n) {
		u64 const r(g->reference_positions[n]), a(g->aligned_positions[n]);
		if (r > ref_len) return fail(ctx, V2M_ERR_PRECONDITION, "node %llu: reference position %llu is past the reference (%llu)", (unsigned long long) n, (unsigned long long) r, (unsigned long long) ref_len);
		if (n) {
			u64 const pr(g->reference_positions[n - 1]), pa(g->aligned_positions[n - 1]);
			if (r <= pr) return fail(ctx, V2M_ERR_PRECONDITION, "reference positions must increase strictly (node %llu)", (unsigned long long) n);
			if (a < pa || a - pa < r - pr)
				return fail(ctx, V2M_ERR_PRECONDITION, "node %llu: aligned distance is shorter than the reference distance", (unsigned long long) n);
		}
		ref_pos[n] = u32(r);
		aln_pos[n] = u32(a);
	}
	if (0 != g->alt_edge_count_csum[0] || E != g->alt_edge_count_csum[N])
		return fail(ctx, V2M_ERR_PRECONDITION, "alt_edge_count_csum must run from 0 to edge_count");
	for (u64 n(0); n <= N; ++n) {
		if (n && g->alt_edge_count_csum[n] < g->alt_edge_count_csum[n - 1]) return fail(ctx, V2M_ERR_PRECONDITION, "alt_edge_count_csum decreases at node %llu", (unsigned long long) n);
		csum[n] = u32(g->alt_edge_count_csum[n]);
	}
	if (N >= 1 && csum[N] != csum[N - 1])
		return fail(ctx, V2M_ERR_PRECONDITION, "the sink node cannot have ALT edges");

	std::vector<v2m::edge_span> spans(E);
	std::vector<v2m::edge_patch> patches(E);
	std::vector<u32> tgt_prefix_max(E + 1, 0);
	std::vector<u64> overlappable((E + 63) / 64, 0);
	u64 label_total(0);
	if (E) {
		label_total = g->alt_edge_label_offsets[E];
		if (label_total >= limit32) return fail(ctx, V2M_ERR_UNSUPPORTED, "label pool too large");
		if (label_total && !g->alt_edge_label_bytes) return fail(ctx, V2M_ERR_INVALID_ARGUMENT, "alt_edge_label_bytes is NULL");
		if (0 != g->alt_edge_label_offsets[0]) return fail(ctx, V2M_ERR_PRECONDITION, "alt_edge_label_offsets must start at 0");
	}
	for (u64 n(0); n < N; ++n) {
		for (u32 e(csum[n]); e < csum[n + 1]; ++e) {
			u64 const tgt(g->alt_edge_targets[e]);
			if (tgt <= n || tgt >= N) return fail(ctx, V2M_ERR_PRECONDITION, "edge %u: target %llu must lie after its source node %llu", e, (unsigned long long) tgt, (unsigned long long) n);
			u64 const lo(g->alt_edge_label_offsets[e]), hi(g->alt_edge_label_offsets[e + 1]);
			if (hi < lo || hi > label_total) return fail(ctx, V2M_ERR_PRECONDITION, "edge %u: bad label offsets", e);
			if (hi - lo > u64(aln_pos[tgt]) - aln_pos[n])
				return fail(ctx, V2M_ERR_PRECONDITION, "edge %u: label (%llu) is longer than the aligned span (%u)", e, (unsigned long long) (hi - lo), aln_pos[tgt] - aln_pos[n]);
			spans[e] = {u32(n), u32(tgt)};
			patches[e] = {aln_pos[n], aln_pos[tgt], u32(lo), u32(hi - lo)};
			tgt_prefix_max[e + 1] = std::max(tgt_prefix_max[e], u32(tgt));
			if (n < tgt_prefix_max[e]) overlappable[e >> 6] |= u64(1) << (e & 63);
		}
	}

	std::vector<u32> ovl_rank(overlappable.size() + 1, 0);
	std::vector<u64> blocker_masks;
	for (u64 wi(0); wi < overlappable.size(); ++wi) {
		ovl_rank[wi] = u32(blocker_masks.size());
		for (u64 m(overlappable[wi]); m; m &= m - 1) {
			u64 const b(u64(__builtin_ctzll(m))), e(wi * 64 + b);
			u64 mask(0);
			if (tgt_prefix_max[wi * 64] > spans[e].src) mask = ~u64(0);
			else for (u64 k(0); k < b; ++k) if (spans[wi * 64 + k].tgt > spans[e].src) mask |= u64(1) << k;
			blocker_masks.push_back(mask);
		}
	}
	ovl_rank.back() = u32(blocker_masks.size());

	u32 const n_tiles(u32(std::max<u64>(1, (L + v2m::kTileBytes - 1) / v2m::kTileBytes)));
	std::vector<u32> tile_edge_begin(n_tiles + 1), cross_offsets(n_tiles + 1, 0), cross_edges;
	{
		u32 e(0);
		for (u32 t(0); t <= n_tiles; ++t) {
			u64 const base(u64(t) * v2m::kTileBytes);
			while (e < E && patches[e].aln_begin < base) ++e;
			tile_edge_begin[t] = e;
		}
		tile_edge_begin[n_tiles] = u32(E);
		std::vector<u32> counts(n_tiles + 1, 0);
		auto for_each_crossing = [&](auto &&fn) {
			for (u32 e2(0); e2 < E; ++e2) {
				u64 const first(u64(patches[e2].aln_begin) / v2m::kTileBytes + 1);
				if (0 == patches[e2].aln_end) continue;
				u64 const last((u64(patches[e2].aln_end) - 1) / v2m::kTileBytes);
				for (u64 t(first); t <= last && t < n_tiles; ++t) fn(u32(t), e2);
			}
		};
		for_each_crossing([&](u32 t, u32) { ++counts[t]; });
		for (u32 t(0); t < n_tiles; ++t) cross_offsets[t + 1] = cross_offsets[t] + counts[t];
		cross_edges.resize(cross_offsets[n_tiles]);
		std::vector<u32> cursor(cross_offsets.begin(), cross_offsets.end() - 1);
		for_each_crossing([&](u32 t, u32 e2) { cross_edges[cursor[t]++] = e2; });
	}

	ctx->has_graph = false;
	ctx->windowed = false;
	ctx->has_set = false;
	ctx->n_nodes = N; ctx->n_edges = E; ctx->ref_len = ref_len; ctx->aligned_len = L; ctx->label_bytes = label_total;
	V2M_HIP_TRY(ctx, ctx->d_ref.ensure(std::max<u64>(ref_len, 16)));
	if (ref_len) V2M_HIP_TRY(ctx, hipMemcpyAsync(ctx->d_ref.p, ref_seq, ref_len, hipMemcpyHostToDevice, ctx->stream));
	V2M_HIP_TRY(ctx, ctx->d_labels.ensure(std::max<u64>(label_total, 16)));
	if (label_total) V2M_HIP_TRY(ctx, hipMemcpyAsync(ctx->d_labels.p, g->alt_edge_label_bytes, label_total, hipMemcpyHostToDevice, ctx->stream));
	if (int const rc = upload_vec(ctx, ctx->d_ref_pos, ref_pos)) return rc;
	if (int const rc = upload_vec(ctx, ctx->d_aln_pos, aln_pos)) return rc;
	if (int const rc = upload_vec(ctx, ctx->d_spans, spans)) return rc;
	if (int const rc = upload_vec(ctx, ctx->d_patches, patches)) return rc;
	if (int const rc = upload_vec(ctx, ctx->d_overlappable, overlappable)) return rc;
	if (int const rc = upload_vec(ctx, ctx->d_ovl_rank, ovl_rank)) return rc;
	if (int const rc = upload_vec(ctx, ctx->d_blocker_masks, blocker_masks)) return rc;

	row_view &v(ctx->whole);
	v.begin = 0;
	v.end = L;
	v.max_unaligned = ref_len + label_total;
	v.n_tiles = n_tiles;
	v.has_template0 = false;
	v.words = {0, 0, (E + 63) / 64, (((E + 63) / 64) + 15) & ~u64(15)};
	if (int const rc = upload_vec(ctx, v.d_edge_begin, tile_edge_begin)) return rc;
	if (int const rc = upload_vec(ctx, v.d_cross_offsets, cross_offsets)) return rc;
	if (int const rc = upload_vec(ctx, v.d_cross_edges, cross_edges)) return rc;
	if (int const rc = expand_reference(ctx, v, v.d_template, '-')) return rc;

	ctx->d_paths = nullptr;
	ctx->by_edge_valid = false;
	ctx->path_rows = ctx->path_cols = ctx->path_pitch = 0;
	if (g->paths_by_chrom_copy_and_edge) {
		size_t const bytes(g->path_rows / 64 * g->path_cols * sizeof(u64));
		V2M_HIP_TRY(ctx, ctx->owned_paths.ensure(std::max<size_t>(bytes, 16)));
		if (bytes) V2M_HIP_TRY(ctx, hipMemcpyAsync(ctx->owned_paths.p, g->paths_by_chrom_copy_and_edge, bytes, hipMemcpyHostToDevice, ctx->stream));
		ctx->d_paths = ctx->owned_paths.as<u64>();
		ctx->path_rows = g->path_rows;
		ctx->path_cols = g->path_cols;
		ctx->path_pitch = g->path_rows / 64;
	}
	V2M_HIP_TRY(ctx, hipStreamSynchronize(ctx->stream));

	ctx->has_nul_byte = (ref_len && std::memchr(ref_seq, 0, ref_len)) || (label_total && std::memchr(g->alt_edge_label_bytes, 0, label_total));
	ctx->h_csum = std::move(csum);
	ctx->h_tgt_prefix_max = std::move(tgt_prefix_max);
	ctx->h_aln_pos = std::move(aln_pos);
	ctx->h_patches = std::move(patches);
	ctx->h_overlappable = std::move(overlappable);
	ctx->h_tile_edge_begin = std::move(tile_edge_begin);
	ctx->h_cross_offsets = std::move(cross_offsets);
	ctx->h_cross_edges = std::move(cross_edges);
	ctx->has_graph = true;
	return V2M_OK;
}

int v2m_set_paths_device(v2m_ctx *ctx, const void *d_words, uint64_t path_rows, uint64_t path_cols)
{
	if (!ctx) return V2M_ERR_INVALID_ARGUMENT;
	if (!ctx->has_graph) return fail(ctx, V2M_ERR_STATE, "no graph uploaded");
	if (path_rows % 64 || path_cols % 64 || path_rows < ctx->n_edges)
		return fail(ctx, V2M_ERR_PRECONDITION, "path matrix must be (>= edge_count) x copies with both dimensions multiples of 64");
	if (path_rows && path_cols && (!d_words || ((uintptr_t) d_words & 7))) return fail(ctx, V2M_ERR_INVALID_ARGUMENT, "d_words must be a non-NULL 8-byte aligned device pointer");
	ctx->d_paths = static_cast<u64 const *>(d_words);
	ctx->by_edge_valid = false;
	ctx->path_rows = path_rows;
	ctx->path_cols = path_cols;
	ctx->path_pitch = path_rows / 64;
	return V2M_OK;
}

namespace {

u64 aligned_pitch(u64 words) { return (words + 15) & ~u64(15); }

int transpose_into_owned_paths(v2m_ctx *ctx, u64 const *d_src, u64 n_rows, u64 n_cols, u64 src_pitch)
{
	u64 const pitch(aligned_pitch(n_cols / 64));
	V2M_HIP_TRY(ctx, ctx->owned_paths.ensure(pitch * n_rows * sizeof(u64)));
	if (int const rc = launch_transpose(ctx, d_src, n_rows, n_cols, ctx->owned_paths.as<u64>(), src_pitch, pitch)) return rc;
	ctx->d_paths = ctx->owned_paths.as<u64>();
	ctx->by_edge_valid = false;
	ctx->path_rows = n_cols;
	ctx->path_cols = n_rows;
	ctx->path_pitch = pitch;
	return V2M_OK;
}

}

int v2m_bind_path_matrix_device(v2m_ctx *ctx, const void *d_paths_by_edge_and_chrom_copy, uint64_t n_rows, uint64_t n_cols)
{
	if (!ctx) return V2M_ERR_INVALID_ARGUMENT;
	if (!ctx->has_graph) return fail(ctx, V2M_ERR_STATE, "no graph uploaded");
	if (n_rows % 64 || n_cols % 64)
		return fail(ctx, V2M_ERR_PRECONDITION, "matrix dimensions must be multiples of 64 (got %llu x %llu)", (unsigned long long) n_rows, (unsigned long long) n_cols);
	if (n_cols < ctx->n_edges) return fail(ctx, V2M_ERR_PRECONDITION, "path matrix has %llu edge columns, the graph %llu edges", (unsigned long long) n_cols, (unsigned long long) ctx->n_edges);
	V2M_HIP_TRY(ctx, hipSetDevice(ctx->device));
	ctx->d_paths = nullptr;
	ctx->by_edge_valid = false;
	ctx->path_rows = ctx->path_cols = ctx->path_pitch = 0;
	if (0 == n_rows || 0 == n_cols) return V2M_OK;
	if (!d_paths_by_edge_and_chrom_copy || ((uintptr_t) d_paths_by_edge_and_chrom_copy & 7)) return fail(ctx, V2M_ERR_INVALID_ARGUMENT, "the matrix must be a non-NULL 8-byte aligned device pointer");
	return transpose_into_owned_paths(ctx, static_cast<u64 const *>(d_paths_by_edge_and_chrom_copy), n_rows, n_cols, 0);
}

int v2m_upload_path_slice(v2m_ctx *ctx, const uint64_t *src_words, uint64_t n_rows, uint64_t n_cols, uint64_t first_copy, uint64_t n_copies)
{
	if (!ctx) return V2M_ERR_INVALID_ARGUMENT;
	if (first_copy > n_rows || n_copies > n_rows - first_copy) return fail(ctx, V2M_ERR_INVALID_ARGUMENT, "copies [%llu, %llu) are outside the matrix (%llu rows)", (unsigned long long) first_copy, (unsigned long long) (first_copy + n_copies), (unsigned long long) n_rows);
	u64 const block((n_copies + 7) & ~u64(7));
	return v2m_upload_path_blocks(ctx, src_words, n_rows, n_cols, first_copy, std::max<u64>(block, 8), std::max<u64>(block, 8), first_copy + n_copies);
}

int v2m_upload_path_blocks(v2m_ctx *ctx, const uint64_t *src_words, uint64_t n_rows, uint64_t n_cols, uint64_t first_copy, uint64_t block_copies, uint64_t stride_copies, uint64_t copy_end)
{
	if (!ctx) return V2M_ERR_INVALID_ARGUMENT;
	if (!ctx->has_graph) return fail(ctx, V2M_ERR_STATE, "no graph uploaded");
	if (n_rows % 64 || n_cols % 64)
		return fail(ctx, V2M_ERR_PRECONDITION, "matrix dimensions must be multiples of 64 (got %llu x %llu)", (unsigned long long) n_rows, (unsigned long long) n_cols);
	if (n_cols < ctx->n_edges) return fail(ctx, V2M_ERR_PRECONDITION, "path matrix has %llu edge columns, the graph %llu edges", (unsigned long long) n_cols, (unsigned long long) ctx->n_edges);
	if (first_copy % 8 || block_copies % 8 || stride_copies % 8 || 0 == block_copies || stride_copies < block_copies)
		return fail(ctx, V2M_ERR_INVALID_ARGUMENT, "first_copy, block_copies and stride_copies must be multiples of 8 (whole bytes of the bit-packed columns), 0 < block_copies <= stride_copies");
	if (copy_end > n_rows) return fail(ctx, V2M_ERR_INVALID_ARGUMENT, "copies up to %llu are outside the matrix (%llu rows)", (unsigned long long) copy_end, (unsigned long long) n_rows);
	V2M_HIP_TRY(ctx, hipSetDevice(ctx->device));
	ctx->d_paths = nullptr;
	ctx->by_edge_valid = false;
	ctx->path_rows = ctx->path_cols = ctx->path_pitch = 0;

	u64 n_copies(0), n_blocks(0);
	for (u64 c(first_copy); c < copy_end; c += stride_copies, ++n_blocks) n_copies += std::min(block_copies, copy_end - c);
	if (0 == n_copies || 0 == n_cols) return V2M_OK;
	if (!src_words) return fail(ctx, V2M_ERR_INVALID_ARGUMENT, "NULL matrix pointer");

	u64 const hp((n_copies + 63) / 64 * 64);
	size_t const take((n_copies + 7) / 8), src_col_bytes(n_rows / 8), block_bytes(block_copies / 8), stride_bytes(stride_copies / 8);
	bool const whole(take == src_col_bytes && 1 == n_blocks);
	u64 const src_pitch(whole ? hp / 64 : aligned_pitch(hp / 64));
	size_t const col_bytes(src_pitch * 8), bytes(col_bytes * n_cols);
	V2M_HIP_TRY(ctx, ctx->d_slice_src.ensure(bytes));
	char const *const src(reinterpret_cast<char const *>(src_words) + first_copy / 8);
	if (whole) {
		V2M_HIP_TRY(ctx, hipMemcpyAsync(ctx->d_slice_src.p, src_words, bytes, hipMemcpyHostToDevice, ctx->stream));
	} else {
		unsigned char const tail_mask((n_copies % 8) ? (unsigned char) ((1u << (n_copies % 8)) - 1) : (unsigned char) 0xFF);
		size_t const slot_cols(std::max<size_t>(1, std::min<size_t>(n_cols, (size_t(64) << 20) / col_bytes)));
		if (int const rc = ensure_host_slots(ctx, 2, slot_cols * col_bytes)) return rc;
		scoped_events sent;
		V2M_HIP_TRY(ctx, sent.create(2));
		size_t slot_index(0);
		for (size_t c0(0); c0 < n_cols; c0 += slot_cols, ++slot_index) {
			size_t const nc(std::min(slot_cols, size_t(n_cols) - c0));
			int const b(int(slot_index & 1));
			if (slot_index >= 2) V2M_HIP_TRY(ctx, hipEventSynchronize(sent[b]));
			char *const stage(ctx->host_slots[b]->host.as<char>());
			V2M_POISON_HOST(stage, nc * col_bytes);
			auto const pack([&](size_t lo, size_t hi) {
				for (size_t c(lo); c < hi; ++c) {
					char *const d(stage + c * col_bytes);
					char const *const column(src + (c0 + c) * src_col_bytes);
					size_t done(0);
					for (u64 j(0); j < n_blocks; ++j) {
						size_t const n(std::min(block_bytes, take - done));
						std::memcpy(d + done, column + j * stride_bytes, n);
						done += n;
					}
					d[take - 1] = char((unsigned char) d[take - 1] & tail_mask);
					if (take < col_bytes) std::memset(d + take, 0, col_bytes - take);
				}
			});
			unsigned const n_threads(unsigned(std::max<size_t>(1, std::min<size_t>(8, nc * col_bytes >> 22))));
			if (n_threads <= 1) pack(0, nc);
			else {
				std::vector<std::thread> pool;
				for (unsigned t(0); t < n_threads; ++t) pool.emplace_back(pack, nc * t / n_threads, nc * (t + 1) / n_threads);
				for (auto &t : pool) t.join();
			}
			V2M_HIP_TRY(ctx, hipMemcpyAsync(static_cast<char *>(ctx->d_slice_src.p) + c0 * col_bytes, stage, nc * col_bytes, hipMemcpyHostToDevice, ctx->stream));
			V2M_HIP_TRY(ctx, hipEventRecord(sent[b], ctx->stream));
		}
	}
	if (int const rc = transpose_into_owned_paths(ctx, ctx->d_slice_src.as<u64>(), hp, n_cols, src_pitch)) return rc;
	V2M_HIP_TRY(ctx, hipStreamSynchronize(ctx->stream));
	ctx->d_slice_src.reset();
	return V2M_OK;
}

uint64_t v2m_aligned_length(const v2m_ctx *ctx) { return (ctx && ctx->has_graph) ? ctx->aligned_len : 0; }
uint64_t v2m_min_row_pitch(const v2m_ctx *ctx) { return (ctx && ctx->has_graph) ? ((ctx->view().length() + 255) & ~u64(255)) : 0; }
uint64_t v2m_max_unaligned_length(const v2m_ctx *ctx) { return (ctx && ctx->has_graph) ? ctx->view().max_unaligned : 0; }
uint64_t v2m_window_length(const v2m_ctx *ctx) { return (ctx && ctx->has_graph) ? ctx->view().length() : 0; }

namespace {

struct window_tile_tables {
	std::vector<u32> edge_begin, edge_end, cross_offsets{0}, cross_edges;
	u32 n_tiles() const { return u32(edge_end.size()); }
};

u32 first_edge_beginning_at(v2m_ctx const *ctx, u64 col)
{
	auto const &patches(ctx->h_patches);
	return u32(std::partition_point(patches.begin(), patches.end(), [&](v2m::edge_patch const &p) { return p.aln_begin < col; }) - patches.begin());
}

void append_window_tiles(v2m_ctx const *ctx, u64 col_begin, u64 col_end, window_tile_tables &tb)
{
	auto const &patches(ctx->h_patches);
	u64 const n_tiles((col_end - col_begin + v2m::kTileBytes - 1) / v2m::kTileBytes);
	u32 begin(first_edge_beginning_at(ctx, col_begin));
	for (u64 t(0); t < n_tiles; ++t) {
		u64 const B(col_begin + t * v2m::kTileBytes), T(B / v2m::kTileBytes);
		u32 const end(first_edge_beginning_at(ctx, std::min<u64>(B + v2m::kTileBytes, col_end)));
		for (u32 i(ctx->h_cross_offsets[T]); i < ctx->h_cross_offsets[T + 1]; ++i)
			if (patches[ctx->h_cross_edges[i]].aln_end > B) tb.cross_edges.push_back(ctx->h_cross_edges[i]);
		for (u32 e(ctx->h_tile_edge_begin[T]); e < begin; ++e)
			if (patches[e].aln_end > B) tb.cross_edges.push_back(e);
		tb.edge_begin.push_back(begin);
		tb.edge_end.push_back(end);
		tb.cross_offsets.push_back(u32(tb.cross_edges.size()));
		begin = end;
	}
}

u64 first_edge_reaching_past(v2m_ctx const *ctx, u64 col_begin, u32 e_hi)
{
	u64 e_lo(0), hi(e_hi);
	while (e_lo < hi) {
		u64 const mid((e_lo + hi) / 2);
		if (ctx->h_aln_pos[ctx->h_tgt_prefix_max[mid + 1]] > col_begin) hi = mid; else e_lo = mid + 1;
	}
	return e_lo;
}

word_range words_of_edges(v2m_ctx const *ctx, u64 e_lo, u64 e_hi)
{
	u64 restart(0), lo(0), word_hi(0);
	if (e_lo < e_hi) {
		lo = e_lo / 64;
		word_hi = (e_hi + 63) / 64;
		restart = lo;
		while (restart > 0 && (ctx->h_overlappable[restart] & 1)) --restart;
	}
	return {restart, lo, word_hi, (word_hi - restart + 15) & ~u64(15)};
}

}


int v2m_set_column_window(v2m_ctx *ctx, uint64_t col_begin, uint64_t col_end)
{
	if (!ctx) return V2M_ERR_INVALID_ARGUMENT;
	if (!ctx->has_graph) return fail(ctx, V2M_ERR_STATE, "no graph uploaded");
	u64 const L(ctx->aligned_len);
	if (!(col_begin < col_end && col_end <= L))
		return fail(ctx, V2M_ERR_INVALID_ARGUMENT, "column window [%llu, %llu) is empty or not within the aligned length %llu",
			(unsigned long long) col_begin, (unsigned long long) col_end, (unsigned long long) L);
	ctx->windowed = false;
	if (0 == col_begin && L == col_end) return V2M_OK;
	V2M_HIP_TRY(ctx, hipSetDevice(ctx->device));

	window_tile_tables tb;
	append_window_tiles(ctx, col_begin, col_end, tb);
	u32 const e_hi(tb.edge_end.back());
	tb.edge_begin.push_back(e_hi);
	row_view &w(ctx->window);
	w.words = words_of_edges(ctx, first_edge_reaching_past(ctx, col_begin, e_hi), e_hi);
	w.begin = col_begin;
	w.end = col_end;
	w.max_unaligned = col_end - col_begin;
	w.n_tiles = u32(tb.edge_end.size());
	w.has_template0 = false;
	if (int const rc = upload_vec(ctx, w.d_edge_begin, tb.edge_begin)) return rc;
	if (int const rc = upload_vec(ctx, w.d_cross_offsets, tb.cross_offsets)) return rc;
	if (int const rc = upload_vec(ctx, w.d_cross_edges, tb.cross_edges)) return rc;
	if (int const rc = expand_reference(ctx, w, w.d_template, '-')) return rc;
	V2M_HIP_TRY(ctx, hipStreamSynchronize(ctx->stream));
	ctx->windowed = true;
	return V2M_OK;
}

// ... 35 lines not shown
}

struct scoped_set_call {
	v2m_ctx *ctx;
	explicit scoped_set_call(v2m_ctx *c) : ctx(c) { c->set_call = true; }
	~scoped_set_call() { ctx->set_call = false; }
};

int check_set_call(v2m_ctx *ctx, v2m_row_batch const *rows, u32 flags)
{
	if (int const rc = check_batch(ctx, rows, flags)) return rc;
	if (!ctx->has_set) return fail(ctx, V2M_ERR_STATE, "no window set (v2m_set_window_set)");
	if (flags & V2M_SPLICE_BGZF) return fail(ctx, V2M_ERR_UNSUPPORTED, "V2M_SPLICE_BGZF is not supported by the window-set calls");
	return V2M_OK;
}

}

int v2m_set_window_set(v2m_ctx *ctx, uint64_t n_windows, const uint64_t *col_begin, const uint64_t *col_end)
{
	if (!ctx) return V2M_ERR_INVALID_ARGUMENT;
	if (!ctx->has_graph) return fail(ctx, V2M_ERR_STATE, "no graph uploaded");
	if (0 == n_windows) return fail(ctx, V2M_ERR_INVALID_ARGUMENT, "a window set needs at least one window");
	if (!col_begin || !col_end) return fail(ctx, V2M_ERR_INVALID_ARGUMENT, "NULL array");
	u64 const L(ctx->aligned_len);
	u64 n_tiles(0);
	for (u64 k(0); k < n_windows; ++k) {
		if (!(col_begin[k] < col_end[k] && col_end[k] <= L))
			return fail(ctx, V2M_ERR_INVALID_ARGUMENT, "window %llu, [%llu, %llu), is empty or not within the aligned length %llu",
				(unsigned long long) k, (unsigned long long) col_begin[k], (unsigned long long) col_end[k], (unsigned long long) L);
		n_tiles += (col_end[k] - col_begin[k] + v2m::kTileBytes - 1) / v2m::kTileBytes;
	}
	std::vector<u64> slot_offset(n_windows);
	u64 pitch(0);
	if (int const rc = v2m_window_set_layout(n_windows, col_begin, col_end, slot_offset.data(), &pitch)) return fail(ctx, rc, "%s", g_create_error.c_str());
	if (n_windows >= 0xFFFFFFFFull || n_tiles >= 0x7FFFFFFFull)
		return fail(ctx, V2M_ERR_UNSUPPORTED, "the window set has too many tiles (%llu) for one set: split it", (unsigned long long) n_tiles);
	ctx->has_set = false;
	V2M_HIP_TRY(ctx, hipSetDevice(ctx->device));

	auto &set(ctx->set);
	window_tile_tables tb;
	std::vector<u32> tile_col_begin, tile_col_end, tile_record_offset, tile_window, first_tile(n_windows + 1), slot_offset32(n_windows);
	tile_col_begin.reserve(n_tiles); tile_col_end.reserve(n_tiles); tile_record_offset.reserve(n_tiles); tile_window.reserve(n_tiles);
	set.lengths.resize(n_windows);
	u64 e_lo(~u64(0)), e_hi(0), slots_end(0);
	for (u64 k(0); k < n_windows; ++k) {
		u64 const len(col_end[k] - col_begin[k]);
		first_tile[k] = tb.n_tiles();
		slot_offset32[k] = u32(slot_offset[k]);
		set.lengths[k] = u32(len);
		slots_end = slot_offset[k] + ((len + 15) & ~u64(15));
		append_window_tiles(ctx, col_begin[k], col_end[k], tb);
		for (u64 j(0); j * v2m::kTileBytes < len; ++j) {
			tile_col_begin.push_back(u32(col_begin[k] + j * v2m::kTileBytes));
			tile_col_end.push_back(u32(std::min<u64>(col_begin[k] + (j + 1) * v2m::kTileBytes, col_end[k])));
			tile_record_offset.push_back(u32(slot_offset[k] + j * v2m::kTileBytes));
			tile_window.push_back(u32(k));
		}
		u32 const w_hi(tb.edge_end.back());
		u64 const w_lo(first_edge_reaching_past(ctx, col_begin[k], w_hi));
		if (w_lo < w_hi) { e_lo = std::min(e_lo, w_lo); e_hi = std::max<u64>(e_hi, w_hi); }
	}
	first_tile[n_windows] = tb.n_tiles();
	tb.edge_begin.push_back(0);
	row_view &v(set.view);
	v.words = words_of_edges(ctx, std::min(e_lo, e_hi), e_hi);
	v.begin = 0;
	v.end = slots_end;
	v.max_unaligned = slots_end;
	v.n_tiles = tb.n_tiles();
	v.has_template0 = false;
	set.n_windows = n_windows;
	set.pitch = pitch;
	u64 total(0);
	for (u32 const len : set.lengths) total += len;
	set.mean_tile_bytes = std::max<u64>(1, total / v.n_tiles);
	if (int const rc = upload_vec(ctx, v.d_edge_begin, tb.edge_begin)) return rc;
	if (int const rc = upload_vec(ctx, v.d_cross_offsets, tb.cross_offsets)) return rc;
	if (int const rc = upload_vec(ctx, v.d_cross_edges, tb.cross_edges)) return rc;
	if (int const rc = upload_vec(ctx, set.d_edge_end, tb.edge_end)) return rc;
	if (int const rc = upload_vec(ctx, set.d_col_begin, tile_col_begin)) return rc;
	if (int const rc = upload_vec(ctx, set.d_col_end, tile_col_end)) return rc;
	if (int const rc = upload_vec(ctx, set.d_record_offset, tile_record_offset)) return rc;
	if (int const rc = upload_vec(ctx, set.d_tile_window, tile_window)) return rc;
	if (int const rc = upload_vec(ctx, set.d_first_tile, first_tile)) return rc;
	if (int const rc = upload_vec(ctx, set.d_slot_offset32, slot_offset32)) return rc;
	if (int const rc = expand_reference_set(ctx, v.d_template, '-')) return rc;
	V2M_HIP_TRY(ctx, hipStreamSynchronize(ctx->stream));
	ctx->has_set = true;
	return V2M_OK;
}

int v2m_splice_window_set(v2m_ctx *ctx, const v2m_row_batch *rows, uint32_t flags, v2m_window_sink_fn sink, void *user)
{
	if (int const rc = check_set_call(ctx, rows, flags)) return rc;
	if (!sink) return fail(ctx, V2M_ERR_INVALID_ARGUMENT, "sink is NULL");
	if (0 == rows->n_rows) return V2M_OK;
	V2M_HIP_TRY(ctx, hipSetDevice(ctx->device));
	scoped_set_call const in_set(ctx);
	u64 const n_windows(ctx->set.n_windows);
	return splice_rows_pipeline(ctx, rows, flags & V2M_SPLICE_UNALIGNED, 2, "v2m_splice_window_set", [&](v2m_row_hold &, slot_rows const &sl) -> int {
		for (u64 r(sl.r0); r < sl.r1; ++r)
			if (sink(user, r, sl.row(r), sl.set_lengths ? sl.set_lengths + (r - sl.r0) * n_windows : ctx->set.lengths.data()))
				return fail(ctx, V2M_ERR_SINK, "sink aborted at row %llu", (unsigned long long) r);
		return V2M_OK;
	});
}

int v2m_splice_window_set_device(v2m_ctx *ctx, const v2m_row_batch *rows, uint32_t flags, void *d_out, uint64_t record_pitch, uint32_t *lengths_out)
{
	if (int const rc = check_set_call(ctx, rows, flags)) return rc;
	if (0 == rows->n_rows) return V2M_OK;
	if (!d_out || ((uintptr_t) d_out & 15)) return fail(ctx, V2M_ERR_INVALID_ARGUMENT, "d_out must be a 16-byte aligned device pointer");
	if (record_pitch % 16 || record_pitch < ctx->set.view.end)
		return fail(ctx, V2M_ERR_INVALID_ARGUMENT, "record_pitch must be a multiple of 16 and at least the end of the last slot, %llu", (unsigned long long) ctx->set.view.end);
	V2M_HIP_TRY(ctx, hipSetDevice(ctx->device));
	scoped_set_call const in_set(ctx);
	u64 const n_windows(ctx->set.n_windows);
	if (!(flags & V2M_SPLICE_UNALIGNED)) {
		if (int const rc = splice_aligned_slice(ctx, rows, 0, rows->n_rows, static_cast<char *>(d_out), record_pitch)) return rc;
		if (lengths_out)
			for (u64 r(0); r < rows->n_rows; ++r) std::copy(ctx->set.lengths.begin(), ctx->set.lengths.end(), lengths_out + r * n_windows);
		return V2M_OK;
	}
	ctx->set_lengths_slot = 0;
	if (int const rc = splice_unaligned_slice(ctx, rows, 0, rows->n_rows, static_cast<char *>(d_out), record_pitch)) return rc;
	if (lengths_out) {
		V2M_HIP_TRY(ctx, hipMemcpyAsync(lengths_out, ctx->d_set_lengths[0].p, rows->n_rows * n_windows * sizeof(u32), hipMemcpyDeviceToHost, ctx->stream));
		V2M_HIP_TRY(ctx, hipStreamSynchronize(ctx->stream));
	}
	return V2M_OK;
}



namespace {

int pbwt_check_state(v2m_ctx *ctx, uint64_t n_copies, uint64_t n_chunks, const uint32_t *start_order, int max_copies)
{
	if (0 == n_copies || n_copies > u64(max_copies)) return fail(ctx, V2M_ERR_UNSUPPORTED, "this GPU chunk walk holds at most %d chromosome copies (got %llu)", max_copies, (unsigned long long) n_copies);
	if (n_copies > ctx->path_cols) return fail(ctx, V2M_ERR_INVALID_ARGUMENT, "the bound path matrix has %llu copies, %llu asked for", (unsigned long long) ctx->path_cols, (unsigned long long) n_copies);
	if (ctx->path_cols > u64(max_copies)) return fail(ctx, V2M_ERR_UNSUPPORTED, "this GPU chunk walk reads edge columns of at most %d copies; the bound path matrix has %llu columns", max_copies, (unsigned long long) ctx->path_cols);
	if (ctx->n_edges >= 0x7FFFFFF0ull) return fail(ctx, V2M_ERR_UNSUPPORTED, "the GPU chunk walk keeps edge indices in 31 bits (the graph has %llu edges)", (unsigned long long) ctx->n_edges);
	for (u64 i(0), n(n_chunks * n_copies); i < n; ++i)
		if (start_order[i] >= n_copies) return fail(ctx, V2M_ERR_INVALID_ARGUMENT, "start_order[%llu] = %u is not a chromosome copy (%llu copies)", (unsigned long long) i, start_order[i], (unsigned long long) n_copies);
	return V2M_OK;
}

int edge_major_paths(v2m_ctx *ctx, u64 const **d_by_edge_out)
{
	u64 const rows(ctx->path_rows), cols(ctx->path_cols);
	if (!ctx->by_edge_valid) {
		V2M_HIP_TRY(ctx, ctx->d_by_edge.ensure(std::max<size_t>(16, rows * (cols / 64) * sizeof(u64))));
		if (int const rc = launch_transpose(ctx, ctx->d_paths, rows, cols, ctx->d_by_edge.as<u64>(), ctx->path_pitch, 0)) return rc;
		ctx->by_edge_valid = true;
	}
	*d_by_edge_out = ctx->d_by_edge.as<u64>();
	return V2M_OK;
}

int pbwt_cut_trials_impl(v2m_ctx *ctx, uint64_t n_copies, uint64_t min_distance,
	uint64_t n_candidates, const uint32_t *cand_edge, const uint64_t *cand_aligned_pos,
	uint64_t n_chunks, const uint64_t *chunk_first, const uint32_t *start_order, const uint32_t *start_divergence,
	uint64_t trial_capacity, uint32_t *trial_pred, uint32_t *trial_class_count, uint64_t *trial_end, uint32_t *chunk_status,
	v2m_trials_sink sink, void *sink_user)
{
	if (!ctx) return V2M_ERR_INVALID_ARGUMENT;
	if (!ctx->has_graph || !ctx->d_paths) return fail(ctx, V2M_ERR_STATE, "the founder search needs an uploaded graph with its path matrix");
	if (0 == n_chunks) return V2M_OK;
	if (!cand_edge || !cand_aligned_pos || !chunk_first || !start_order || !start_divergence || (!sink && (!trial_pred || !trial_class_count)) || !trial_end || !chunk_status)
		return fail(ctx, V2M_ERR_INVALID_ARGUMENT, "NULL array");
	if (int const rc = pbwt_check_state(ctx, n_copies, n_chunks, start_order, v2m::kPbwtMaxCopies)) return rc;
	if (n_candidates >= 0xFFFFFFFFull || ctx->n_edges >= 0xFFFFFFFDull) return fail(ctx, V2M_ERR_UNSUPPORTED, "candidate and edge indices are kept in 32 bits");
	if (chunk_first[0] < 1 || chunk_first[n_chunks] > n_candidates) return fail(ctx, V2M_ERR_INVALID_ARGUMENT, "chunk bounds outside the candidate list");
	for (u64 k(0); k < n_chunks; ++k) if (chunk_first[k] > chunk_first[k + 1]) return fail(ctx, V2M_ERR_INVALID_ARGUMENT, "chunk bounds must not decrease");
	for (u64 c(0); c < n_candidates; ++c) {
		if (cand_edge[c] > ctx->n_edges || (c && cand_edge[c] < cand_edge[c - 1])) return fail(ctx, V2M_ERR_INVALID_ARGUMENT, "candidate edges must ascend and stay inside the graph (candidate %llu)", (unsigned long long) c);
		if (c && cand_aligned_pos[c] < cand_aligned_pos[c - 1]) return fail(ctx, V2M_ERR_INVALID_ARGUMENT, "candidate aligned positions must not decrease (candidate %llu)", (unsigned long long) c);
	}
	V2M_HIP_TRY(ctx, hipSetDevice(ctx->device));

	u64 const cols(ctx->path_cols);
	u64 const *d_by_edge(nullptr);
	if (int const rc = edge_major_paths(ctx, &d_by_edge)) return rc;
	dev_buf d_first, d_cand_edge, d_cand_aln, d_chunk_first, d_order, d_div, d_pred, d_class, d_end, d_status;

	auto const up([&](dev_buf &dst, void const *src, size_t bytes) -> int {
		V2M_HIP_TRY(ctx, dst.ensure(std::max<size_t>(bytes, 16)));
		if (bytes) V2M_HIP_TRY(ctx, hipMemcpyAsync(dst.p, src, bytes, hipMemcpyHostToDevice, ctx->stream));
		return V2M_OK;
	});
	if (int const rc = up(d_cand_edge, cand_edge, n_candidates * sizeof(u32))) return rc;
	if (int const rc = up(d_cand_aln, cand_aligned_pos, n_candidates * sizeof(u64))) return rc;
	if (int const rc = up(d_chunk_first, chunk_first, (n_chunks + 1) * sizeof(u64))) return rc;
	if (int const rc = up(d_order, start_order, n_chunks * n_copies * sizeof(u32))) return rc;
	if (int const rc = up(d_div, start_divergence, n_chunks * n_copies * sizeof(u32))) return rc;
	u32 const n_edges(u32(ctx->n_edges));
	V2M_HIP_TRY(ctx, d_first.ensure((u64(n_edges) + 1) * sizeof(u32)));
	V2M_HIP_TRY(ctx, d_pred.ensure(std::max<u64>(16, n_chunks * trial_capacity * sizeof(u32))));
	V2M_HIP_TRY(ctx, d_class.ensure(std::max<u64>(16, n_chunks * trial_capacity * sizeof(u32))));
	V2M_HIP_TRY(ctx, d_end.ensure(n_candidates * sizeof(u64)));
	V2M_HIP_TRY(ctx, d_status.ensure(n_chunks * sizeof(u32)));
	V2M_HIP_TRY(ctx, hipMemsetAsync(d_status.p, 0xFF, n_chunks * sizeof(u32), ctx->stream));
	hipLaunchKernelGGL(v2m::pbwt_first_candidate_kernel, dim3(unsigned((u64(n_edges) + 1 + 255) / 256)), dim3(256), 0, ctx->stream,
		d_cand_edge.as<u32>(), u32(n_candidates), n_edges, d_first.as<u32>());
	auto const launch_trials([&](auto per_tag) {
		hipLaunchKernelGGL((v2m::pbwt_cut_trials_kernel<decltype(per_tag)::value>), dim3(unsigned(n_chunks)), dim3(v2m::kPbwtThreads), 0, ctx->stream,
			d_by_edge, u32(cols / 64), u32(n_copies), n_edges, d_first.as<u32>(), d_cand_edge.as<u32>(), d_cand_aln.as<u64>(), min_distance,
			d_chunk_first.as<u64>(), d_order.as<u32>(), d_div.as<u32>(), trial_capacity, d_pred.as<u32>(), d_class.as<u32>(), d_end.as<u64>(), d_status.as<u32>());
	});
	pbwt_dispatch_per_thread<v2m::kPbwtPerThread>(ctx->path_cols, launch_trials);
	V2M_HIP_TRY(ctx, hipGetLastError());
	V2M_HIP_TRY(ctx, hipMemcpyAsync(chunk_status, d_status.p, n_chunks * sizeof(u32), hipMemcpyDeviceToHost, ctx->stream));
	u64 const cand_lo(chunk_first[0]), cand_hi(chunk_first[n_chunks]);
	if (cand_hi > cand_lo) V2M_HIP_TRY(ctx, hipMemcpyAsync(trial_end + cand_lo, d_end.as<u64>() + cand_lo, (cand_hi - cand_lo) * sizeof(u64), hipMemcpyDeviceToHost, ctx->stream));
	V2M_HIP_TRY(ctx, hipStreamSynchronize(ctx->stream));
	std::vector<u64> produced(n_chunks, 0);
	for (u64 k(0); k < n_chunks; ++k) {
		if (0 != chunk_status[k] || chunk_first[k] == chunk_first[k + 1]) { if (0 != chunk_status[k]) chunk_status[k] = 1; continue; }
		u64 const n(trial_end[chunk_first[k + 1] - 1]);
		if (n > trial_capacity) { chunk_status[k] = 1; continue; }
		produced[k] = n;
	}
	if (!sink) {
		for (u64 k(0); k < n_chunks; ++k) {
			if (0 == produced[k]) continue;
			V2M_HIP_TRY(ctx, hipMemcpyAsync(trial_pred + k * trial_capacity, d_pred.as<u32>() + k * trial_capacity, produced[k] * sizeof(u32), hipMemcpyDeviceToHost, ctx->stream));
			V2M_HIP_TRY(ctx, hipMemcpyAsync(trial_class_count + k * trial_capacity, d_class.as<u32>() + k * trial_capacity, produced[k] * sizeof(u32), hipMemcpyDeviceToHost, ctx->stream));
		}
		V2M_HIP_TRY(ctx, hipStreamSynchronize(ctx->stream));
		return V2M_OK;
	}

	u64 const slot_pairs(std::max<u64>(trial_capacity, u64(4) << 20));
	for (auto &slot : ctx->trials_stage) V2M_HIP_TRY(ctx, slot.ensure(2 * slot_pairs * sizeof(u32)));
	scoped_events ev;
	V2M_HIP_TRY(ctx, ev.create(2));
	struct slice { u64 first, end; };
	std::vector<slice> slices;
	for (u64 k(0); k < n_chunks;) {
		u64 end(k), pairs(0);
		while (end < n_chunks && (end == k || pairs + produced[end] <= slot_pairs)) pairs += produced[end++];
		slices.push_back({k, end});
		k = end;
	}
	auto const issue([&](std::size_t i) -> int {
		u32 *const pred(ctx->trials_stage[i & 1].as<u32>()), *const cls(pred + slot_pairs);
		V2M_POISON_HOST(pred, 2 * slot_pairs * sizeof(u32));
		u64 at(0);
		for (u64 k(slices[i].first); k < slices[i].end; ++k) {
			if (0 == produced[k]) continue;
			V2M_HIP_TRY(ctx, hipMemcpyAsync(pred + at, d_pred.as<u32>() + k * trial_capacity, produced[k] * sizeof(u32), hipMemcpyDeviceToHost, ctx->stream));
			V2M_HIP_TRY(ctx, hipMemcpyAsync(cls + at, d_class.as<u32>() + k * trial_capacity, produced[k] * sizeof(u32), hipMemcpyDeviceToHost, ctx->stream));
			at += produced[k];
		}
		V2M_HIP_TRY(ctx, hipEventRecord(ev[i & 1], ctx->stream));
		return V2M_OK;
	});
	if (int const rc = issue(0)) return rc;
	for (std::size_t i(0); i < slices.size(); ++i) {
		if (i + 1 < slices.size()) if (int const rc = issue(i + 1)) return rc;
		V2M_HIP_TRY(ctx, hipEventSynchronize(ev[i & 1]));
		u32 const *const pred(ctx->trials_stage[i & 1].as<u32>()), *const cls(pred + slot_pairs);
		u64 at(0);
		for (u64 k(slices[i].first); k < slices[i].end; ++k) {
			if (int const rc = sink(sink_user, k, chunk_status[k], pred + at, cls + at, produced[k])) {
				(void) hipStreamSynchronize(ctx->stream);
				return fail(ctx, V2M_ERR_SINK, "the trial sink returned %d at chunk %llu", rc, (unsigned long long) k);
			}
			at += produced[k];
		}
	}
	return V2M_OK;
}

}


int v2m_pbwt_cut_trials(v2m_ctx *ctx, uint64_t n_copies, uint64_t min_distance,
	uint64_t n_candidates, const uint32_t *cand_edge, const uint64_t *cand_aligned_pos,
	uint64_t n_chunks, const uint64_t *chunk_first, const uint32_t *start_order, const uint32_t *start_divergence,
	uint64_t trial_capacity, uint32_t *trial_pred, uint32_t *trial_class_count, uint64_t *trial_end, uint32_t *chunk_status)
{
	return pbwt_cut_trials_impl(ctx, n_copies, min_distance, n_candidates, cand_edge, cand_aligned_pos, n_chunks, chunk_first, start_order, start_divergence,
		trial_capacity, trial_pred, trial_class_count, trial_end, chunk_status, nullptr, nullptr);
}


int v2m_pbwt_cut_trials_streamed(v2m_ctx *ctx, uint64_t n_copies, uint64_t min_distance,
	uint64_t n_candidates, const uint32_t *cand_edge, const uint64_t *cand_aligned_pos,
	uint64_t n_chunks, const uint64_t *chunk_first, const uint32_t *start_order, const uint32_t *start_divergence,
	uint64_t trial_capacity, uint64_t *trial_end, uint32_t *chunk_status, v2m_trials_sink sink, void *sink_user)
{
	if (ctx && !sink) return fail(ctx, V2M_ERR_INVALID_ARGUMENT, "NULL sink");
	return pbwt_cut_trials_impl(ctx, n_copies, min_distance, n_candidates, cand_edge, cand_aligned_pos, n_chunks, chunk_first, start_order, start_divergence,
		trial_capacity, nullptr, nullptr, trial_end, chunk_status, sink, sink_user);
}


int v2m_pbwt_cut_records(v2m_ctx *ctx, uint64_t n_copies, uint64_t n_cuts, const uint32_t *cut_edge,
	uint64_t n_chunks, const uint64_t *chunk_first_cut, const uint32_t *start_edge, const uint32_t *start_order, const uint32_t *start_divergence,
	uint64_t pool_capacity, uint32_t *pool_lhs, uint32_t *pool_rhs, uint32_t *pool_size,
	uint64_t *rec_pool_end, uint32_t *rec_distinct, uint32_t *rec_first_class, uint32_t *rec_first_is_ref, uint32_t *chunk_status)
{
	if (!ctx) return V2M_ERR_INVALID_ARGUMENT;
// ... 816 lines not shown
```

Before: 6933.

## Resolve effective edges in place at bind time with an undo log

```diff
diff --git a/vcf2multialign_amd/csrc/kernels.hpp b/vcf2multialign_amd/csrc/kernels.hpp
--- a/vcf2multialign_amd/csrc/kernels.hpp
+++ b/vcf2multialign_amd/csrc/kernels.hpp
@@ -917,6 +917,50 @@
 constexpr u32 kResolveQueueShards = 1024;
 constexpr u32 kMaxBackWords = 2048;
 
+struct path_fix { u64 index, raw, effective; };
+struct path_fix_log {
+	path_fix *entries;
+	u32 *count;
+	u32 capacity;
+};
+
+template <bool kInPlace> struct path_words { typedef u64 const *__restrict__ type; };
+template <> struct path_words<true> { typedef u64 const *type; };
+template <bool kInPlace> struct eff_words { typedef u64 *__restrict__ type; };
+template <> struct eff_words<true> { typedef u64 *type; };
+
+template <bool kInPlace>
+__device__ __forceinline__ void store_effective_word(u64 *eff, u64 index, u64 raw, u64 value, path_fix_log const &log)
+{
+	if (!kInPlace) { eff[index] = value; return; }
+	bool const changed = value != raw;
+	u64 const lanes = __ballot(changed);
+	if (!changed) return;
+	int const lane = threadIdx.x & 63, leader = __builtin_ctzll(lanes);
+	u32 base = 0;
+	if (lane == leader) base = atomicAdd(log.count, (u32) __builtin_popcountll(lanes));
+	base = __shfl(base, leader, kWave);
+	u32 const slot = base + (u32) __builtin_popcountll(lanes & ((1ULL << lane) - 1));
+	if (slot >= log.capacity) return;
+	log.entries[slot] = path_fix{index, raw, value};
+	eff[index] = value;
+}
+
+__global__ __launch_bounds__(256) void apply_path_fixes_kernel(u64 *__restrict__ paths, path_fix const *__restrict__ entries, u32 n, bool to_effective)
+{
+	for (u32 i = blockIdx.x * blockDim.x + threadIdx.x; i < n; i += gridDim.x * blockDim.x) {
+		path_fix const f = entries[i];
+		paths[f.index] = to_effective ? f.effective : f.raw;
+	}
+}
+
+__global__ __launch_bounds__(256) void identity_segments_kernel(u32 *__restrict__ seg_offsets, u32 *__restrict__ seg_edge_begin, u32 *__restrict__ seg_copy, u32 n)
+{
+	u32 const i = blockIdx.x * blockDim.x + threadIdx.x;
+	if (i <= n) seg_offsets[i] = i;
+	if (i < n) { seg_edge_begin[i] = 0; seg_copy[i] = i; }
+}
+
 __device__ __forceinline__ u64 resolve_word_exact(
 	u64 const *__restrict__ paths, u64 words_per_copy, row_segments const &rs, u32 row, u32 s_begin, u32 s_end,
 	edge_span const *__restrict__ spans, u64 const *__restrict__ overlappable,
@@ -969,12 +1013,14 @@
 	return out;
 }
 
+template <bool kInPlace = false>
 __global__ __launch_bounds__(256) void resolve_effective_edges_kernel(
-	u64 const *__restrict__ paths, u64 words_per_copy, u32 n_edges,
+	typename path_words<kInPlace>::type paths, u64 words_per_copy, u32 n_edges,
 	row_segments rs, edge_span const *__restrict__ spans, u64 const *__restrict__ overlappable,
 	u32 const *__restrict__ ovl_rank, u64 const *__restrict__ blocker_masks,
-	u64 *__restrict__ eff, u32 n_words, u32 eff_words_per_row, u32 row_base, u32 word_base,
-	u32 *__restrict__ queue, u32 *__restrict__ queue_counts , u32 shard_capacity, u32 *__restrict__ needs_serial, u32 max_back_words)
+	typename eff_words<kInPlace>::type eff, u32 n_words, u32 eff_words_per_row, u32 row_base, u32 word_base,
+	u32 *__restrict__ queue, u32 *__restrict__ queue_counts , u32 shard_capacity, u32 *__restrict__ needs_serial, u32 max_back_words,
+	path_fix_log log = path_fix_log{})
 {
 	u32 const row = blockIdx.x + row_base;
 	u32 const shard = (blockIdx.y * gridDim.x + blockIdx.x) % kResolveQueueShards;
@@ -989,6 +1035,7 @@
 	}
 	u32 const w_first = word_base + blockIdx.y * kResolveWordsPerThread * blockDim.x + threadIdx.x;
 	u64 w_all[kResolveWordsPerThread], ovl_all[kResolveWordsPerThread], mask_a[kResolveWordsPerThread], mask_b[kResolveWordsPerThread];
+	u64 raw_tail = 0;
 	u32 rank_all[kResolveWordsPerThread];
 #pragma unroll
 	for (int piece = 0; piece < kResolveWordsPerThread; ++piece) {
@@ -997,7 +1044,7 @@
 		w_all[piece] = row_words ? row_words[wc] : 0;
 		ovl_all[piece] = overlappable[wc];
 		rank_all[piece] = ovl_rank[wc];
-		if (wi == (n_edges - 1) >> 6) w_all[piece] &= tail_mask;
+		if (wi == (n_edges - 1) >> 6) { raw_tail = w_all[piece]; w_all[piece] &= tail_mask; }
 	}
 #pragma unroll
 	for (int piece = 0; piece < kResolveWordsPerThread; ++piece) {
@@ -1015,7 +1062,9 @@
 		bool const in_range = wi < n_words;
 		u64 const w = w_all[piece], ov = w & ovl_all[piece], ov2 = ov & (ov - 1);
 		bool const hard = in_range && ov && ((w & mask_a[piece]) || (ov2 && ((w & mask_b[piece]) || (ov2 & (ov2 - 1)))));
-		if (in_range && !hard) eff[(u64) row * eff_words_per_row + wi] = w;
+		if (!kInPlace) { if (in_range && !hard) eff[(u64) row * eff_words_per_row + wi] = w; }
+		else if (wi == (n_edges - 1) >> 6 && !hard && w != raw_tail)
+			store_effective_word<kInPlace>(eff, (u64) row * eff_words_per_row + wi, raw_tail, w, log);
 		u64 const hard_lanes = __ballot(hard);
 		if (hard_lanes) {
 			u32 base = 0;
@@ -1024,17 +1073,20 @@
 			if (hard) {
 				u32 const slot = base + __builtin_amdgcn_mbcnt_hi((u32) (hard_lanes >> 32), __builtin_amdgcn_mbcnt_lo((u32) hard_lanes, 0));
 				if (slot < shard_capacity) queue[(u64) shard * shard_capacity + slot] = (row - row_base) * n_words + wi;
-				else eff[(u64) row * eff_words_per_row + wi] = resolve_word_exact(paths, words_per_copy, rs, row, s_begin, s_end, spans, overlappable, wi, w, ovl_all[piece], needs_serial, max_back_words);
-			}
-		}
-	}
-}
-
+				else store_effective_word<kInPlace>(eff, (u64) row * eff_words_per_row + wi, (kInPlace && wi == (n_edges - 1) >> 6) ? raw_tail : w,
+					resolve_word_exact(paths, words_per_copy, rs, row, s_begin, s_end, spans, overlappable, wi, w, ovl_all[piece], needs_serial, max_back_words), log);
+			}
+		}
+	}
+}
+
+template <bool kInPlace = false>
 __global__ __launch_bounds__(256) void resolve_queued_words_kernel(
-	u64 const *__restrict__ paths, u64 words_per_copy, u32 n_edges,
+	typename path_words<kInPlace>::type paths, u64 words_per_copy, u32 n_edges,
 	row_segments rs, edge_span const *__restrict__ spans, u64 const *__restrict__ overlappable,
-	u64 *__restrict__ eff, u32 n_words, u32 eff_words_per_row, u32 row_base,
-	u32 const *__restrict__ queue, u32 const *__restrict__ queue_counts, u32 shard_capacity, u32 *__restrict__ needs_serial, u32 max_back_words)
+	typename eff_words<kInPlace>::type eff, u32 n_words, u32 eff_words_per_row, u32 row_base,
+	u32 const *__restrict__ queue, u32 const *__restrict__ queue_counts, u32 shard_capacity, u32 *__restrict__ needs_serial, u32 max_back_words,
+	path_fix_log log = path_fix_log{})
 {
 	u32 const shard = blockIdx.x % kResolveQueueShards, part = blockIdx.x / kResolveQueueShards, parts = gridDim.x / kResolveQueueShards;
 	u32 const n = queue_counts[shard] < shard_capacity ? queue_counts[shard] : shard_capacity;
@@ -1044,17 +1096,21 @@
 		u32 const row = row_base + entry / n_words, wi = entry % n_words;
 		u32 const s_begin = rs.seg_offsets[row], s_end = rs.seg_offsets[row + 1];
 		u64 w = load_row_word(paths, words_per_copy, rs, row, s_begin, s_end, wi);
+		u64 const raw = w;
 		if (wi == (n_edges - 1) >> 6) w &= tail_mask;
-		eff[(u64) row * eff_words_per_row + wi] = resolve_word_exact(paths, words_per_copy, rs, row, s_begin, s_end, spans, overlappable, wi, w, overlappable[wi], needs_serial, max_back_words);
-	}
-}
-
-
+		store_effective_word<kInPlace>(eff, (u64) row * eff_words_per_row + wi, raw,
+			resolve_word_exact(paths, words_per_copy, rs, row, s_begin, s_end, spans, overlappable, wi, w, overlappable[wi], needs_serial, max_back_words), log);
+	}
+}
+
+
+template <bool kInPlace = false>
 __global__ __launch_bounds__(256) void resolve_rows_serial_kernel(
-	u64 const *__restrict__ paths, u64 words_per_copy, u32 n_edges,
+	typename path_words<kInPlace>::type paths, u64 words_per_copy, u32 n_edges,
 	row_segments rs, edge_span const *__restrict__ spans,
-	u64 *__restrict__ eff, u64 eff_words_per_row, u32 n_rows, u32 const *__restrict__ needs_serial,
-	u32 word_begin , u32 word_end)
+	typename eff_words<kInPlace>::type eff, u64 eff_words_per_row, u32 n_rows, u32 const *__restrict__ needs_serial,
+	u32 word_begin , u32 word_end,
+	path_fix_log log = path_fix_log{})
 {
 	int const lane = threadIdx.x & 63;
 	u32 const row = blockIdx.x * (blockDim.x >> 6) + (threadIdx.x >> 6);
@@ -1063,14 +1119,13 @@
 
 	u32 const s_begin = rs.seg_offsets[row], s_end = rs.seg_offsets[row + 1];
 	u32 const n_words = (n_edges + 63) / 64;
-	u64 *const eff_row = eff + (u64) row * eff_words_per_row;
 	u32 cur = 0;
 
 	for (u32 base = word_begin; base < word_end; base += 64) {
 		u32 const wi = base + lane;
-		u64 w = 0;
+		u64 w = 0, raw = 0;
 		if (wi < word_end) {
-			w = load_row_word(paths, words_per_copy, rs, row, s_begin, s_end, wi);
+			raw = w = load_row_word(paths, words_per_copy, rs, row, s_begin, s_end, wi);
 			if (wi == n_words - 1 && (n_edges & 63))
 				w &= (1ULL << (n_edges & 63)) - 1;
 		}
@@ -1125,7 +1180,7 @@
 			cur = chunk_max > cur ? chunk_max : cur;
 		}
 		if (wi < word_end)
-			eff_row[wi] = out;
+			store_effective_word<kInPlace>(eff, (u64) row * eff_words_per_row + wi, raw, out, log);
 	}
 }
 
diff --git a/vcf2multialign_amd/csrc/v2m_hip.hip b/vcf2multialign_amd/csrc/v2m_hip.hip
--- a/vcf2multialign_amd/csrc/v2m_hip.hip
+++ b/vcf2multialign_amd/csrc/v2m_hip.hip
@@ -197,6 +197,15 @@
 	u64 path_pitch{};
 	dev_buf d_by_edge;
 	bool by_edge_valid{};
+	bool paths_effective{};
+	bool fix_valid{};
+	bool fix_pending{};
+	u64 fix_count{}, fix_capacity{};
+	u64 lead_zero_words{};
+	dev_buf d_fix_log, d_fix_count, d_bind_segments;
+	u64 bind_segment_rows{};
+	pinned_buf h_fix_count;
+	hipEvent_t ev_fix{};
 
 	struct transpose_pick { u64 rows, cols, src_pitch, dst_pitch; std::string kernel; };
 	std::vector<transpose_pick> transpose_choice;
@@ -750,6 +759,163 @@
 }
 
 
+
+u32 max_back_words_knob()
+{
+	char const *const back_env(std::getenv("V2M_MAX_BACK_WORDS"));
+	return (back_env && *back_env) ? u32(std::strtoul(back_env, nullptr, 10)) : v2m::kMaxBackWords;
+}
+
+int ensure_owned_paths(v2m_ctx *ctx, u64 pitch, u64 n_copies)
+{
+	size_t const before(ctx->owned_paths.bytes);
+	V2M_HIP_TRY(ctx, ctx->owned_paths.ensure(std::max<size_t>(pitch * (n_copies + 1) * sizeof(u64), 16)));
+	if (before != ctx->owned_paths.bytes) ctx->lead_zero_words = 0;
+	if (pitch > ctx->lead_zero_words) {
+		V2M_HIP_TRY(ctx, hipMemsetAsync(ctx->owned_paths.p, 0, pitch * sizeof(u64), ctx->stream));
+		ctx->lead_zero_words = pitch;
+	}
+	return V2M_OK;
+}
+
+void drop_path_fixes(v2m_ctx *ctx)
+{
+	ctx->paths_effective = ctx->fix_valid = ctx->fix_pending = false;
+	ctx->fix_count = 0;
+}
+
+int apply_path_fixes(v2m_ctx *ctx, u64 n, bool to_effective)
+{
+	if (n) {
+		timed_launch tl(ctx, V2M_KERNEL_RESOLVE);
+		hipLaunchKernelGGL(v2m::apply_path_fixes_kernel, dim3(unsigned(std::min<u64>((n + 255) / 256, 1024))), dim3(256), 0, ctx->stream,
+			ctx->owned_paths.as<u64>() + ctx->path_pitch, ctx->d_fix_log.as<v2m::path_fix>(), u32(n), to_effective);
+	}
+	V2M_HIP_TRY(ctx, hipGetLastError());
+	return V2M_OK;
+}
+
+int settle_path_fixes(v2m_ctx *ctx)
+{
+	if (!ctx->fix_pending) return V2M_OK;
+	ctx->fix_pending = false;
+	V2M_HIP_TRY(ctx, hipEventSynchronize(ctx->ev_fix));
+	u64 const wanted(*ctx->h_fix_count.as<u32>());
+	if (wanted > ctx->fix_capacity) {
+		ctx->paths_effective = ctx->fix_valid = false;
+		return apply_path_fixes(ctx, ctx->fix_capacity, false);
+	}
+	ctx->fix_count = wanted;
+	ctx->fix_valid = ctx->paths_effective = true;
+	return V2M_OK;
+}
+
+int paths_to_raw(v2m_ctx *ctx)
+{
+	if (int const rc = settle_path_fixes(ctx)) return rc;
+	if (!ctx->paths_effective) return V2M_OK;
+	ctx->paths_effective = false;
+	return apply_path_fixes(ctx, ctx->fix_count, false);
+}
+
+int paths_to_effective(v2m_ctx *ctx)
+{
+	if (int const rc = settle_path_fixes(ctx)) return rc;
+	if (ctx->paths_effective || !ctx->fix_valid) return V2M_OK;
+	ctx->paths_effective = true;
+	return apply_path_fixes(ctx, ctx->fix_count, true);
+}
+
+int resolve_owned_paths(v2m_ctx *ctx)
+{
+	drop_path_fixes(ctx);
+	char const *const e(std::getenv("V2M_RESOLVE_AT_BIND"));
+	if (e && *e && 0 == std::atoi(e)) return V2M_OK;
+	u64 const n_words((ctx->n_edges + 63) / 64), n_copies(ctx->path_cols), pitch(ctx->path_pitch);
+	if (0 == ctx->n_edges || 0 == n_copies || n_copies > 65535 * 256ull || n_copies * n_words >= 0xFFFFFFFFull) return V2M_OK;
+
+	if (ctx->bind_segment_rows < n_copies) {
+		u64 const n(std::max<u64>(n_copies, 1024));
+		V2M_HIP_TRY(ctx, ctx->d_bind_segments.ensure((3 * n + 1) * sizeof(u32)));
+		u32 *const t(ctx->d_bind_segments.as<u32>());
+		hipLaunchKernelGGL(v2m::identity_segments_kernel, dim3(unsigned(n / 256 + 1)), dim3(256), 0, ctx->stream, t, t + (n + 1), t + (2 * n + 1), u32(n));
+		ctx->bind_segment_rows = n;
+	}
+	u64 const seg_n(ctx->bind_segment_rows);
+	u32 *const seg(ctx->d_bind_segments.as<u32>());
+	v2m::row_segments const rs{seg, seg + (seg_n + 1), seg + (2 * seg_n + 1), nullptr, 0};
+
+	char const *const log_env(std::getenv("V2M_RESOLVE_LOG_CAPACITY"));
+	u64 const capacity((log_env && *log_env) ? std::min<u64>(std::strtoull(log_env, nullptr, 10), 0x7FFFFFFFull) : std::min<u64>(n_copies * n_words / 32 + 4096, 0x7FFFFFFFull));
+	V2M_HIP_TRY(ctx, ctx->d_fix_log.ensure(std::max<size_t>(capacity * sizeof(v2m::path_fix), 16)));
+	V2M_HIP_TRY(ctx, ctx->d_fix_count.ensure(16));
+	V2M_HIP_TRY(ctx, ctx->h_fix_count.ensure(16));
+	ctx->fix_capacity = capacity;
+	v2m::path_fix_log const log{ctx->d_fix_log.as<v2m::path_fix>(), ctx->d_fix_count.as<u32>(), u32(capacity)};
+
+	char const *const capacity_env(std::getenv("V2M_RESOLVE_QUEUE_CAPACITY"));
+	u64 const shard_capacity((capacity_env && *capacity_env) ? std::min<u64>(std::strtoull(capacity_env, nullptr, 10), (u64(1) << 28) / v2m::kResolveQueueShards)
+		: std::max<u64>(256, std::min<u64>(n_copies * n_words / 8, u64(1) << 26) / v2m::kResolveQueueShards));
+	V2M_HIP_TRY(ctx, ctx->d_resolve_queue.ensure(std::max<size_t>(shard_capacity * v2m::kResolveQueueShards * sizeof(u32), 16)));
+	V2M_HIP_TRY(ctx, ctx->d_resolve_count.ensure(v2m::kResolveQueueShards * sizeof(u32)));
+	V2M_HIP_TRY(ctx, ctx->d_needs_serial.ensure(n_copies * sizeof(u32)));
+	V2M_HIP_TRY(ctx, hipMemsetAsync(ctx->d_resolve_count.p, 0, v2m::kResolveQueueShards * sizeof(u32), ctx->stream));
+	V2M_HIP_TRY(ctx, hipMemsetAsync(ctx->d_needs_serial.p, 0, n_copies * sizeof(u32), ctx->stream));
+	V2M_HIP_TRY(ctx, hipMemsetAsync(ctx->d_fix_count.p, 0, sizeof(u32), ctx->stream));
+	u64 *const paths(ctx->owned_paths.as<u64>() + pitch);
+	u32 const max_back_words(max_back_words_knob());
+	{
+		timed_launch tl(ctx, V2M_KERNEL_RESOLVE);
+		for (u64 piece0(0), pieces((n_words + 256 * v2m::kResolveWordsPerThread - 1) / (256 * v2m::kResolveWordsPerThread)); piece0 < pieces; piece0 += 65535)
+			hipLaunchKernelGGL(v2m::resolve_effective_edges_kernel<true>, dim3(unsigned(n_copies), unsigned(std::min<u64>(65535, pieces - piece0))), dim3(256), 0, ctx->stream,
+				paths, pitch, u32(ctx->n_edges), rs, ctx->d_spans.as<v2m::edge_span>(), ctx->d_overlappable.as<u64>(),
+				ctx->d_ovl_rank.as<u32>(), ctx->d_blocker_masks.as<u64>(),
+				paths, u32(n_words), u32(pitch), 0u, u32(piece0 * 256 * v2m::kResolveWordsPerThread),
+				ctx->d_resolve_queue.as<u32>(), ctx->d_resolve_count.as<u32>(), u32(shard_capacity), ctx->d_needs_serial.as<u32>(), max_back_words, log);
+		hipLaunchKernelGGL(v2m::resolve_queued_words_kernel<true>, dim3(2 * v2m::kResolveQueueShards), dim3(256), 0, ctx->stream,
+			paths, pitch, u32(ctx->n_edges), rs, ctx->d_spans.as<v2m::edge_span>(), ctx->d_overlappable.as<u64>(),
+			paths, u32(n_words), u32(pitch), 0u,
+			ctx->d_resolve_queue.as<u32>(), ctx->d_resolve_count.as<u32>(), u32(shard_capacity), ctx->d_needs_serial.as<u32>(), max_back_words, log);
+		hipLaunchKernelGGL(v2m::resolve_rows_serial_kernel<true>, dim3(unsigned((n_copies + 3) / 4)), dim3(256), 0, ctx->stream,
+			paths, pitch, u32(ctx->n_edges), rs, ctx->d_spans.as<v2m::edge_span>(),
+			paths, pitch, u32(n_copies), ctx->d_needs_serial.as<u32>(), 0u, u32(n_words), log);
+	}
+	V2M_HIP_TRY(ctx, hipGetLastError());
+	V2M_HIP_TRY(ctx, hipMemcpyAsync(ctx->h_fix_count.p, ctx->d_fix_count.p, sizeof(u32), hipMemcpyDeviceToHost, ctx->stream));
+	V2M_HIP_TRY(ctx, hipEventRecord(ctx->ev_fix, ctx->stream));
+	ctx->fix_pending = true;
+	return V2M_OK;
+}
+
+bool direct_slice_words(v2m_ctx *ctx, v2m_row_batch const *rows, u64 row_begin, u64 row_end, u64 const *&eff, u64 &stride)
+{
+	if (ctx->set_call || ctx->windowed || !(ctx->fix_pending || ctx->fix_valid) || 0 == ctx->n_edges || !rows->copy_index) return false;
+	if (rows->cut_offsets && rows->cut_offsets[row_end] != rows->cut_offsets[row_begin]) return false;
+	u64 const n_rows(row_end - row_begin);
+	u32 const *const copy(rows->copy_index + row_begin);
+	bool const lead_ref(V2M_PLOIDY_MAX == copy[0]);
+	u64 first(0);
+	if (lead_ref) {
+		bool all_ref(true);
+		for (u64 r(1); r < n_rows && all_ref; ++r) all_ref = V2M_PLOIDY_MAX == copy[r];
+		if (!all_ref) {
+			for (u64 r(1); r < n_rows; ++r) if (copy[r] != r - 1) return false;
+			if (n_rows - 1 > ctx->path_cols) return false;
+		}
+		stride = all_ref ? 0 : ctx->path_pitch;
+	}
+	else {
+		first = copy[0];
+		for (u64 r(1); r < n_rows; ++r) if (copy[r] != first + r) return false;
+		if (first + n_rows > ctx->path_cols) return false;
+		stride = ctx->path_pitch;
+	}
+	if (V2M_OK != paths_to_effective(ctx) || !ctx->paths_effective) return false;
+	eff = ctx->owned_paths.as<u64>() + (lead_ref ? 0 : (first + 1) * ctx->path_pitch);
+	return true;
+}
+
+
 int resolve_slice(v2m_ctx *ctx, v2m_row_batch const *rows, u64 row_begin, u64 row_end)
 {
 	u64 const n_rows(row_end - row_begin);
@@ -779,13 +945,13 @@
 	V2M_HIP_TRY(ctx, hipMemsetAsync(ctx->d_needs_serial.p, 0, n_rows * sizeof(u32), ctx->stream));
 
 	bool const any_switching_row(pr.any_switching_row);
+	if (any_switching_row) if (int const rc = paths_to_raw(ctx)) return rc;
 	if (any_switching_row) V2M_HIP_TRY(ctx, ctx->d_row_bits.ensure(n_rows * eff_words * sizeof(u64)));
 
 	u64 *const d_eff(ctx->d_eff.as<u64>() - wr.restart);
 	u64 *const d_row_bits(any_switching_row ? ctx->d_row_bits.as<u64>() - wr.restart : nullptr);
 	v2m::row_segments rs{ctx->d_seg_offsets.as<u32>(), ctx->d_seg_edge_begin.as<u32>(), ctx->d_seg_copy.as<u32>(), d_row_bits, u32(eff_words)};
-	char const *const back_env(std::getenv("V2M_MAX_BACK_WORDS"));
-	u32 const max_back_words((back_env && *back_env) ? u32(std::strtoul(back_env, nullptr, 10)) : v2m::kMaxBackWords);
+	u32 const max_back_words(max_back_words_knob());
 	char const *const capacity_env(std::getenv("V2M_RESOLVE_QUEUE_CAPACITY"));
 	bool const capacity_forced(capacity_env && *capacity_env);
 	{
@@ -804,19 +970,19 @@
 			V2M_HIP_TRY(ctx, ctx->d_resolve_count.ensure(v2m::kResolveQueueShards * sizeof(u32)));
 			V2M_HIP_TRY(ctx, hipMemsetAsync(ctx->d_resolve_count.p, 0, v2m::kResolveQueueShards * sizeof(u32), ctx->stream));
 			for (u64 piece0(0), pieces((resolved_words + 256 * v2m::kResolveWordsPerThread - 1) / (256 * v2m::kResolveWordsPerThread)); piece0 < pieces; piece0 += 65535)
-				hipLaunchKernelGGL(v2m::resolve_effective_edges_kernel, dim3(unsigned(nr), unsigned(std::min<u64>(65535, pieces - piece0))), dim3(256), 0, ctx->stream,
+				hipLaunchKernelGGL(v2m::resolve_effective_edges_kernel<false>, dim3(unsigned(nr), unsigned(std::min<u64>(65535, pieces - piece0))), dim3(256), 0, ctx->stream,
 					ctx->d_paths, ctx->path_pitch, u32(ctx->n_edges), rs, ctx->d_spans.as<v2m::edge_span>(), ctx->d_overlappable.as<u64>(),
 					ctx->d_ovl_rank.as<u32>(), ctx->d_blocker_masks.as<u64>(),
 					d_eff, u32(n_words), u32(eff_words), u32(r0), u32(wr.lo + piece0 * 256 * v2m::kResolveWordsPerThread),
-					ctx->d_resolve_queue.as<u32>(), ctx->d_resolve_count.as<u32>(), u32(shard_capacity), ctx->d_needs_serial.as<u32>(), max_back_words);
-			hipLaunchKernelGGL(v2m::resolve_queued_words_kernel, dim3(2 * v2m::kResolveQueueShards), dim3(256), 0, ctx->stream,
+					ctx->d_resolve_queue.as<u32>(), ctx->d_resolve_count.as<u32>(), u32(shard_capacity), ctx->d_needs_serial.as<u32>(), max_back_words, v2m::path_fix_log{});
+			hipLaunchKernelGGL(v2m::resolve_queued_words_kernel<false>, dim3(2 * v2m::kResolveQueueShards), dim3(256), 0, ctx->stream,
 				ctx->d_paths, ctx->path_pitch, u32(ctx->n_edges), rs, ctx->d_spans.as<v2m::edge_span>(), ctx->d_overlappable.as<u64>(),
 				d_eff, u32(n_words), u32(eff_words), u32(r0),
-				ctx->d_resolve_queue.as<u32>(), ctx->d_resolve_count.as<u32>(), u32(shard_capacity), ctx->d_needs_serial.as<u32>(), max_back_words);
-		}
-		hipLaunchKernelGGL(v2m::resolve_rows_serial_kernel, dim3(unsigned((n_rows + 3) / 4)), dim3(256), 0, ctx->stream,
+				ctx->d_resolve_queue.as<u32>(), ctx->d_resolve_count.as<u32>(), u32(shard_capacity), ctx->d_needs_serial.as<u32>(), max_back_words, v2m::path_fix_log{});
+		}
+		hipLaunchKernelGGL(v2m::resolve_rows_serial_kernel<false>, dim3(unsigned((n_rows + 3) / 4)), dim3(256), 0, ctx->stream,
 			ctx->d_paths, ctx->path_pitch, u32(ctx->n_edges), rs, ctx->d_spans.as<v2m::edge_span>(),
-			d_eff, eff_words, u32(n_rows), ctx->d_needs_serial.as<u32>(), u32(wr.restart), u32(n_words));
+			d_eff, eff_words, u32(n_rows), ctx->d_needs_serial.as<u32>(), u32(wr.restart), u32(n_words), v2m::path_fix_log{});
 	}
 	V2M_HIP_TRY(ctx, hipGetLastError());
 	return V2M_OK;
@@ -898,9 +1064,15 @@
 {
 	u64 const n_rows(row_end - row_begin);
 	if (0 == n_rows || 0 == ctx->aligned_len) return V2M_OK;
-	if (int const rc = resolve_slice(ctx, rows, row_begin, row_end)) return rc;
-
 	row_view const &v(ctx->view());
+	u64 const *d_eff(nullptr);
+	u64 eff_stride(0);
+	if (!direct_slice_words(ctx, rows, row_begin, row_end, d_eff, eff_stride)) {
+		if (int const rc = resolve_slice(ctx, rows, row_begin, row_end)) return rc;
+		d_eff = ctx->d_eff.as<u64>() - v.words.restart;
+		eff_stride = v.words.stride;
+	}
+
 	splice_grid g;
 	if (int const rc = make_grid(ctx, n_rows, g)) return rc;
 	v2m::tile_tables const tt{v.d_edge_begin.as<u32>(), v.d_cross_offsets.as<u32>(), v.d_cross_edges.as<u32>()};
@@ -908,13 +1080,13 @@
 	auto const launch([&](bool nt) {
 		auto const go([&](auto kernel, auto... window) {
 			hipLaunchKernelGGL(kernel, dim3(unsigned(g.n_blocks)), dim3(v2m::kSpliceThreads), 0, ctx->stream,
-				v.d_template.as<v2m::vec4u>(), ctx->d_eff.as<u64>() - v.words.restart, v.words.stride, tt, ctx->d_patches.as<v2m::edge_patch>(), ctx->d_labels.as<char>(),
+				v.d_template.as<v2m::vec4u>(), d_eff, eff_stride, tt, ctx->d_patches.as<v2m::edge_patch>(), ctx->d_labels.as<char>(),
 				d_out, row_pitch, u32(n_rows), g.rows_per_group, g.n_groups, v.n_tiles, g.tile_run, store_limit, '-', window...);
 		});
 		if (ctx->set_call) {
 			auto const go_set([&](auto kernel) {
 				hipLaunchKernelGGL(kernel, dim3(unsigned(g.n_blocks)), dim3(v2m::kSpliceThreads), 0, ctx->stream,
-					v.d_template.as<v2m::vec4u>(), ctx->d_eff.as<u64>() - v.words.restart, v.words.stride, tt, set_tables(ctx), ctx->d_patches.as<v2m::edge_patch>(), ctx->d_labels.as<char>(),
+					v.d_template.as<v2m::vec4u>(), d_eff, eff_stride, tt, set_tables(ctx), ctx->d_patches.as<v2m::edge_patch>(), ctx->d_labels.as<char>(),
 					d_out, row_pitch, u32(n_rows), g.rows_per_group, g.n_groups, v.n_tiles, g.tile_run, '-');
 			});
 			if (nt) go_set(v2m::splice_aligned_set_kernel<true>);
@@ -946,7 +1118,13 @@
 		if (int const rc = set ? expand_reference_set(ctx, v.d_template0, 0) : expand_reference(ctx, v, v.d_template0, 0)) return rc;
 		v.has_template0 = true;
 	}
-	if (int const rc = resolve_slice(ctx, rows, row_begin, row_end)) return rc;
+	u64 const *d_eff(nullptr);
+	u64 eff_stride(0);
+	if (!direct_slice_words(ctx, rows, row_begin, row_end, d_eff, eff_stride)) {
+		if (int const rc = resolve_slice(ctx, rows, row_begin, row_end)) return rc;
+		d_eff = ctx->d_eff.as<u64>() - v.words.restart;
+		eff_stride = v.words.stride;
+	}
 
 	splice_grid g;
 	if (int const rc = make_grid(ctx, n_rows, g)) return rc;
@@ -957,7 +1135,6 @@
 	}
 	bool const windowed(ctx->windowed);
 	v2m::tile_tables const tt{v.d_edge_begin.as<u32>(), v.d_cross_offsets.as<u32>(), v.d_cross_edges.as<u32>()};
-	u64 const *const d_eff(ctx->d_eff.as<u64>() - v.words.restart);
 	{
 		char const *const ce(std::getenv("V2M_COUNT_ROWS_PER_GROUP"));
 		u32 const count_rows(u32(std::min<u64>(std::max<u64>(1, n_rows), (ce && *ce && std::atoi(ce) > 0) ? u64(std::min(std::atoi(ce), int(v2m::kCountRowsMax))) : u64(v2m::kCountRowsMax))));
@@ -965,12 +1142,12 @@
 		timed_launch tl(ctx, V2M_KERNEL_UNALIGNED_COUNT);
 		auto const count([&](auto kernel, auto... window) {
 			hipLaunchKernelGGL(kernel, dim3(unsigned(u64(v.n_tiles) * count_groups)), dim3(v2m::kSpliceThreads), 0, ctx->stream,
-				v.d_template0.as<v2m::vec4u>(), d_eff, v.words.stride, tt, ctx->d_patches.as<v2m::edge_patch>(), ctx->d_labels.as<char>(),
+				v.d_template0.as<v2m::vec4u>(), d_eff, eff_stride, tt, ctx->d_patches.as<v2m::edge_patch>(), ctx->d_labels.as<char>(),
 				ctx->d_tile_counts.as<u32>(), v.n_tiles, u32(n_rows), count_rows, count_groups, g.tile_run, window...);
 		});
 		if (set)
 			hipLaunchKernelGGL(v2m::count_unaligned_set_kernel, dim3(unsigned(u64(v.n_tiles) * count_groups)), dim3(v2m::kSpliceThreads), 0, ctx->stream,
-				v.d_template0.as<v2m::vec4u>(), d_eff, v.words.stride, tt, set_tables(ctx), ctx->d_patches.as<v2m::edge_patch>(), ctx->d_labels.as<char>(),
+				v.d_template0.as<v2m::vec4u>(), d_eff, eff_stride, tt, set_tables(ctx), ctx->d_patches.as<v2m::edge_patch>(), ctx->d_labels.as<char>(),
 				ctx->d_tile_counts.as<u32>(), v.n_tiles, u32(n_rows), count_rows, count_groups, g.tile_run);
 		else if (windowed) count(v2m::count_unaligned_window_kernel, u32(v.begin), u32(v.end));
 		else count(v2m::count_unaligned_kernel);
@@ -985,13 +1162,13 @@
 	auto const launch([&](bool nt) {
 		auto const go([&](auto kernel, auto... window) {
 			hipLaunchKernelGGL(kernel, dim3(unsigned(g.n_blocks)), dim3(v2m::kSpliceThreads), 0, ctx->stream,
-				v.d_template0.as<v2m::vec4u>(), d_eff, v.words.stride, tt, ctx->d_patches.as<v2m::edge_patch>(), ctx->d_labels.as<char>(),
+				v.d_template0.as<v2m::vec4u>(), d_eff, eff_stride, tt, ctx->d_patches.as<v2m::edge_patch>(), ctx->d_labels.as<char>(),
 				ctx->d_tile_counts.as<u32>(), v.n_tiles, d_out, row_pitch, u32(n_rows), g.rows_per_group, g.n_groups, g.tile_run, window...);
 		});
 		if (set) {
 			auto const go_set([&](auto kernel) {
 				hipLaunchKernelGGL(kernel, dim3(unsigned(g.n_blocks)), dim3(v2m::kSpliceThreads), 0, ctx->stream,
-					v.d_template0.as<v2m::vec4u>(), d_eff, v.words.stride, tt, set_tables(ctx), ctx->d_patches.as<v2m::edge_patch>(), ctx->d_labels.as<char>(),
+					v.d_template0.as<v2m::vec4u>(), d_eff, eff_stride, tt, set_tables(ctx), ctx->d_patches.as<v2m::edge_patch>(), ctx->d_labels.as<char>(),
 					ctx->d_set_tile_offsets.as<u32>(), v.n_tiles, d_out, row_pitch, u32(n_rows), g.rows_per_group, g.n_groups, g.tile_run);
 			});
 			if (nt) go_set(v2m::splice_unaligned_set_kernel<true>);
@@ -1445,6 +1622,7 @@
 		if (hipSuccess == st) st = hipEventCreateWithFlags(&ctx->ev_row_stage[i], hipEventDisableTiming);
 		if (hipSuccess == st) st = hipEventCreateWithFlags(&ctx->ev_inflate_in[i], hipEventDisableTiming);
 	}
+	if (hipSuccess == st) st = hipEventCreateWithFlags(&ctx->ev_fix, hipEventDisableTiming);
 	if (hipSuccess != st) {
 		std::string const what(hipGetErrorString(st));
 		v2m_ctx_destroy(ctx);
@@ -1472,6 +1650,7 @@
 		if (ctx->ev_row_stage[i]) (void) hipEventDestroy(ctx->ev_row_stage[i]);
 		if (ctx->ev_inflate_in[i]) (void) hipEventDestroy(ctx->ev_inflate_in[i]);
 	}
+	if (ctx->ev_fix) (void) hipEventDestroy(ctx->ev_fix);
 	for (auto &slot : ctx->host_slots) if (slot && slot->copied) (void) hipEventDestroy(slot->copied);
 	(void) hipStreamDestroy(ctx->stream);
 	(void) hipStreamDestroy(ctx->copy_stream);
@@ -1671,14 +1850,17 @@
 	ctx->d_paths = nullptr;
 	ctx->by_edge_valid = false;
 	ctx->path_rows = ctx->path_cols = ctx->path_pitch = 0;
+	drop_path_fixes(ctx);
 	if (g->paths_by_chrom_copy_and_edge) {
-		size_t const bytes(g->path_rows / 64 * g->path_cols * sizeof(u64));
-		V2M_HIP_TRY(ctx, ctx->owned_paths.ensure(std::max<size_t>(bytes, 16)));
-		if (bytes) V2M_HIP_TRY(ctx, hipMemcpyAsync(ctx->owned_paths.p, g->paths_by_chrom_copy_and_edge, bytes, hipMemcpyHostToDevice, ctx->stream));
-		ctx->d_paths = ctx->owned_paths.as<u64>();
+		u64 const pitch(g->path_rows / 64);
+		size_t const bytes(pitch * g->path_cols * sizeof(u64));
+		if (int const rc = ensure_owned_paths(ctx, pitch, g->path_cols)) return rc;
+		if (bytes) V2M_HIP_TRY(ctx, hipMemcpyAsync(ctx->owned_paths.as<u64>() + pitch, g->paths_by_chrom_copy_and_edge, bytes, hipMemcpyHostToDevice, ctx->stream));
+		ctx->d_paths = ctx->owned_paths.as<u64>() + pitch;
 		ctx->path_rows = g->path_rows;
 		ctx->path_cols = g->path_cols;
-		ctx->path_pitch = g->path_rows / 64;
+		ctx->path_pitch = pitch;
+		if (int const rc = resolve_owned_paths(ctx)) return rc;
 	}
 	V2M_HIP_TRY(ctx, hipStreamSynchronize(ctx->stream));
 
@@ -1703,6 +1885,7 @@
 		return fail(ctx, V2M_ERR_PRECONDITION, "path matrix must be (>= edge_count) x copies with both dimensions multiples of 64");
 	if (path_rows && path_cols && (!d_words || ((uintptr_t) d_words & 7))) return fail(ctx, V2M_ERR_INVALID_ARGUMENT, "d_words must be a non-NULL 8-byte aligned device pointer");
 	ctx->d_paths = static_cast<u64 const *>(d_words);
+	drop_path_fixes(ctx);
 	ctx->by_edge_valid = false;
 	ctx->path_rows = path_rows;
 	ctx->path_cols = path_cols;
@@ -1717,14 +1900,15 @@
 int transpose_into_owned_paths(v2m_ctx *ctx, u64 const *d_src, u64 n_rows, u64 n_cols, u64 src_pitch)
 {
 	u64 const pitch(aligned_pitch(n_cols / 64));
-	V2M_HIP_TRY(ctx, ctx->owned_paths.ensure(pitch * n_rows * sizeof(u64)));
-	if (int const rc = launch_transpose(ctx, d_src, n_rows, n_cols, ctx->owned_paths.as<u64>(), src_pitch, pitch)) return rc;
-	ctx->d_paths = ctx->owned_paths.as<u64>();
+	drop_path_fixes(ctx);
+	if (int const rc = ensure_owned_paths(ctx, pitch, n_rows)) return rc;
+	if (int const rc = launch_transpose(ctx, d_src, n_rows, n_cols, ctx->owned_paths.as<u64>() + pitch, src_pitch, pitch)) return rc;
+	ctx->d_paths = ctx->owned_paths.as<u64>() + pitch;
 	ctx->by_edge_valid = false;
 	ctx->path_rows = n_cols;
 	ctx->path_cols = n_rows;
 	ctx->path_pitch = pitch;
-	return V2M_OK;
+	return resolve_owned_paths(ctx);
 }
 
 }
@@ -1740,6 +1924,7 @@
 	ctx->d_paths = nullptr;
 	ctx->by_edge_valid = false;
 	ctx->path_rows = ctx->path_cols = ctx->path_pitch = 0;
+	drop_path_fixes(ctx);
 	if (0 == n_rows || 0 == n_cols) return V2M_OK;
 	if (!d_paths_by_edge_and_chrom_copy || ((uintptr_t) d_paths_by_edge_and_chrom_copy & 7)) return fail(ctx, V2M_ERR_INVALID_ARGUMENT, "the matrix must be a non-NULL 8-byte aligned device pointer");
 	return transpose_into_owned_paths(ctx, static_cast<u64 const *>(d_paths_by_edge_and_chrom_copy), n_rows, n_cols, 0);
@@ -1767,6 +1952,7 @@
 	ctx->d_paths = nullptr;
 	ctx->by_edge_valid = false;
 	ctx->path_rows = ctx->path_cols = ctx->path_pitch = 0;
+	drop_path_fixes(ctx);
 
 	u64 n_copies(0), n_blocks(0);
 	for (u64 c(first_copy); c < copy_end; c += stride_copies, ++n_blocks) n_copies += std::min(block_copies, copy_end - c);
@@ -2108,6 +2294,7 @@
 {
 	u64 const rows(ctx->path_rows), cols(ctx->path_cols);
 	if (!ctx->by_edge_valid) {
+		if (int const rc = paths_to_raw(ctx)) return rc;
 		V2M_HIP_TRY(ctx, ctx->d_by_edge.ensure(std::max<size_t>(16, rows * (cols / 64) * sizeof(u64))));
 		if (int const rc = launch_transpose(ctx, ctx->d_paths, rows, cols, ctx->d_by_edge.as<u64>(), ctx->path_pitch, 0)) return rc;
 		ctx->by_edge_valid = true;
```

Result: slower. 6863 (-1.0%).
